# qiukunlong/seeksv

Measured on AMD Instinct MI355X. Metric: BAM records/sec through getclip+getsv, higher is better.
Workload: dtype i32/u8 (fp64 match-rate compare)

## Files before the change

### include/seeksv_hip.h

```cpp
#ifndef SEEKSV_HIP_H_
#define SEEKSV_HIP_H_

#include <stddef.h>
#include <stdint.h>

#ifdef __cplusplus
extern "C" {
#endif

#define SSV_ABI_VERSION 9

typedef enum {
	SSV_OK = 0,
	SSV_E_NODEVICE = -1,
	SSV_E_HIP = -2,
	SSV_E_ARG = -3,
	SSV_E_STATE = -4,
	SSV_E_NOMEM = -5,
	SSV_E_RANGE = -6
} ssv_status;

typedef enum {
	SSV_MEM_HOST = 0,
	SSV_MEM_DEVICE = 1,
	SSV_MEM_PERSISTENT = 2
} ssv_mem;

typedef struct {
	int32_t tid, pos;
	uint16_t flag;
	uint8_t mapq;
	uint8_t xc;
	uint16_t n_cigar;
	uint16_t pad;
	int32_t l_qseq, mtid, mpos, isize;
	uint32_t cigar_off;
	uint32_t cigar_head[5];
	uint64_t seq_off;
} ssv_record;

#define SSV_NO_SEQ UINT64_MAX
typedef struct {
	int64_t n;
	int32_t mem;
	int32_t max_ref_span;
	const int32_t *tid;
	const int32_t *pos;
	const uint16_t *flag;
	const uint8_t *mapq;
	const uint16_t *n_cigar;
	const int32_t *l_qseq;
	const int32_t *mtid;
	const int32_t *mpos;
	const int32_t *isize;
	const uint32_t *cigar_off;
	const uint32_t *cigar;
	const uint8_t *xc;
	const uint64_t *seq_off;
	const uint8_t *seqqual;
	int64_t n_cigar_total;
	int64_t seqqual_bytes;
	const ssv_record *rec;
	const uint8_t *cigar_ends;
	const struct ssv_tid_run *tid_runs;
	int64_t n_tid_runs;
} ssv_batch_t;

typedef struct ssv_tid_run { int64_t first; int32_t tid; int32_t pad; } ssv_tid_run;

typedef struct ssv_ctx ssv_ctx;


int ssv_ctx_create(int device, ssv_ctx **out);
void ssv_ctx_destroy(ssv_ctx *ctx);
int ssv_sync(ssv_ctx *ctx);
const char *ssv_last_error(const ssv_ctx *ctx);
int ssv_abi_version(void);
int ssv_device_count(void);
void *ssv_stream(ssv_ctx *ctx);

int ssv_host_alloc(size_t bytes, void **p);
int ssv_host_free(void *p);
int ssv_host_register(void *p, size_t bytes);
int ssv_host_unregister(void *p);
int ssv_host_bind_near(void *p, size_t bytes, int device);
int ssv_batch_prefetch(ssv_ctx *ctx, const ssv_batch_t *b);
int ssv_batch_prefetch_drop(ssv_ctx *ctx);

int ssv_batch_retain(ssv_ctx *ctx, const ssv_batch_t *device_batch, ssv_batch_t *out);
int ssv_batch_release(ssv_ctx *ctx, ssv_batch_t *retained);


typedef struct {
	double match_rate;
	int32_t min_mapq;
	int32_t save_low_quality;
	int32_t use_ownership;
	int32_t initial_last_tid;
	int32_t own_lo_tid, own_lo_pos;
	int32_t own_hi_tid, own_hi_pos;
} ssv_clip_params;

int ssv_clip_begin(ssv_ctx *ctx, const ssv_clip_params *p);
int ssv_clip_scan(ssv_ctx *ctx, const ssv_batch_t *b);
int ssv_clip_scan_range(ssv_ctx *ctx, const ssv_batch_t *b, int64_t rec_begin, int64_t rec_end);
int ssv_clip_event_count(ssv_ctx *ctx, int64_t *n_events);

typedef struct {
	int32_t tid;
	uint8_t side;
	uint8_t pad[3];
	int64_t first;
} ssv_table_run;

typedef struct {
	int64_t n_clusters;
	int64_t n_events;
	const int32_t *tid;
	const int32_t *pos;
	const uint8_t *side;
	const int32_t *support;
	const int32_t *left_len;
	const int32_t *right_len;
	const uint8_t *qual_missing;
	const uint64_t *str_off;
	const uint8_t *str;
	const uint64_t *cigar_off;
	const int32_t *n_cigar;
	const uint32_t *cigar;
	int32_t seq_packed;
	int32_t qual_bits;
	uint8_t qual_alphabet[64];
	int32_t format;
	int32_t base_bits;
	int32_t len_bytes, support_bytes, ncig_bytes;
	int32_t qual_group;
	const void *c_len;
	const void *c_support;
	const void *c_ncig;
	const uint8_t *c_flags;
	const ssv_table_run *runs;
	int64_t n_runs;
	const uint64_t *base_exc;
	int64_t n_base_exc;
	uint64_t str_bytes;
	uint64_t cigar_ops;
	int64_t support_sum;
	const void *c_cigar;
	int32_t cigar_bytes, pad4;
} ssv_cluster_table;

int ssv_clip_table_format(ssv_ctx *ctx, int format);
int ssv_clip_table_expand(ssv_ctx *ctx, ssv_cluster_table *t, int32_t n_threads);
uint64_t ssv_table_block_bytes3(int64_t n_bases, int32_t base_bits, int32_t qual_bits);
uint64_t ssv_table_block_bytes3g(int64_t n_bases, int32_t base_bits, int32_t qual_bits, int32_t qual_group);
uint64_t ssv_table_block_bytes(int32_t left_len, int32_t right_len);

int ssv_clip_cluster(ssv_ctx *ctx, ssv_cluster_table *out);
int ssv_clip_cluster_async(ssv_ctx *ctx, int64_t *n_clusters, int64_t *n_events);
int ssv_clip_table_wait(ssv_ctx *ctx, ssv_cluster_table *out);
int ssv_clip_table_wait_prev(ssv_ctx *ctx, ssv_cluster_table *out);


int ssv_isize_begin(ssv_ctx *ctx, int32_t min_mapq, int64_t max_pairs);
int ssv_isize_accumulate(ssv_ctx *ctx, const ssv_batch_t *b, int32_t *done);
int ssv_isize_finish(ssv_ctx *ctx, int64_t *n_pairs, int32_t *mean, int32_t *sd);


typedef struct {
	int32_t up_tid;
	int32_t down_tid;
	int32_t up_pos;
	int32_t down_pos;
	int32_t beg;
	int32_t end;
	uint8_t up_strand;
	uint8_t down_strand;
	uint8_t pad[2];
} ssv_junction;

typedef struct {
	int32_t tid;
	int32_t beg;
	int32_t end;
} ssv_interval;

typedef struct {
	const ssv_junction *junctions;
	int64_t n_junctions;
	int32_t mean, sd, times;
	int32_t disc_min_mapq;
	const ssv_interval *windows;
	int64_t n_windows;
	int32_t depth_min_mapq;
	int32_t n_targets;
	const int32_t *target_len;
} ssv_getsv_params;

int ssv_getsv_begin(ssv_ctx *ctx, const ssv_getsv_params *p);
int ssv_getsv_scan(ssv_ctx *ctx, const ssv_batch_t *b);
int ssv_getsv_prime(ssv_ctx *ctx, const ssv_batch_t *b, int32_t *sufficient);
int ssv_getsv_finish(ssv_ctx *ctx, int32_t *counts,
                     const ssv_interval *ranges, int64_t n_ranges, uint64_t *range_sum,
                     const ssv_interval *points, int64_t n_points, int32_t *point_depth,
                     int32_t *max_depth);

typedef struct ssv_group ssv_group;
int ssv_group_create(ssv_ctx **ctxs, int n, ssv_group **out);
void ssv_group_destroy(ssv_group *g);
int ssv_group_uses_rccl(const ssv_group *g);
int ssv_group_allgather(ssv_group *g, int rank, const void *send, size_t bytes, void *recv);


typedef struct {
	uint64_t c_off;
	uint32_t c_len;
	uint32_t u_len;
} ssv_bgzf_block;

typedef struct {
	int64_t n_records;
// ... 121 lines not shown
```

### seeksv_amd/_abi.py

```python
import ctypes as C
import os

import numpy as np

_HERE = os.path.dirname(os.path.abspath(__file__))
LIBDIR = os.environ.get("SSV_LIBDIR") or os.path.join(_HERE, "lib")

NO_SEQ = (1 << 64) - 1
MEM_HOST, MEM_DEVICE, MEM_PERSISTENT = 0, 1, 2
RECORD_DTYPE = np.dtype([("tid", np.int32), ("pos", np.int32), ("flag", np.uint16), ("mapq", np.uint8), ("xc", np.uint8), ("n_cigar", np.uint16), ("pad", np.uint16),
                         ("l_qseq", np.int32), ("mtid", np.int32), ("mpos", np.int32), ("isize", np.int32), ("cigar_off", np.uint32), ("cigar_head", np.uint32, (5,)),
                         ("seq_off", np.uint64)])
assert RECORD_DTYPE.itemsize == 64


class Batch(C.Structure):
    _fields_ = [
        ("n", C.c_int64), ("mem", C.c_int32), ("max_ref_span", C.c_int32),
        ("tid", C.c_void_p), ("pos", C.c_void_p), ("flag", C.c_void_p), ("mapq", C.c_void_p),
        ("n_cigar", C.c_void_p), ("l_qseq", C.c_void_p), ("mtid", C.c_void_p), ("mpos", C.c_void_p),
        ("isize", C.c_void_p), ("cigar_off", C.c_void_p), ("cigar", C.c_void_p), ("xc", C.c_void_p),
        ("seq_off", C.c_void_p), ("seqqual", C.c_void_p),
        ("n_cigar_total", C.c_int64), ("seqqual_bytes", C.c_int64),
        ("rec", C.c_void_p), ("cigar_ends", C.c_void_p),
        ("tid_runs", C.c_void_p), ("n_tid_runs", C.c_int64),
    ]

    def set_tid_runs(self, runs):
        if runs is None or len(runs) == 0:
            self.tid_runs, self.n_tid_runs, self._runs = None, 0, None
        else:
            self._runs = np.ascontiguousarray(runs, dtype=TID_RUN_DTYPE)
            self.tid_runs, self.n_tid_runs = self._runs.ctypes.data, len(self._runs)

    def get_tid_runs(self):
        if not self.tid_runs or self.n_tid_runs <= 0:
            return None
        return np.frombuffer((C.c_uint8 * (16 * self.n_tid_runs)).from_address(self.tid_runs), dtype=TID_RUN_DTYPE).copy()


TID_RUN_DTYPE = np.dtype([("first", np.int64), ("tid", np.int32), ("pad", np.int32)])


def runs_of_tid(tid):
    tid = np.asarray(tid)
    if tid.size == 0:
        return np.zeros(0, TID_RUN_DTYPE)
    starts = np.concatenate(([0], np.flatnonzero(tid[1:] != tid[:-1]) + 1))
    r = np.zeros(len(starts), TID_RUN_DTYPE)
    r["first"], r["tid"] = starts, tid[starts]
    return r


def rebase_runs(runs, first, n):
    if runs is None or len(runs) == 0 or n <= 0:
        return None
    k0 = int(np.searchsorted(runs["first"], first, side="right")) - 1
    k1 = int(np.searchsorted(runs["first"], first + n, side="left"))
    r = runs[k0:k1].copy()
    r["first"] = np.maximum(r["first"] - first, 0)
    return r


BATCH_FIELDS = [
    ("tid", np.int32), ("pos", np.int32), ("flag", np.uint16), ("mapq", np.uint8), ("n_cigar", np.uint16),
    ("l_qseq", np.int32), ("mtid", np.int32), ("mpos", np.int32), ("isize", np.int32),
    ("cigar_off", np.uint32), ("cigar", np.uint32), ("xc", np.uint8), ("seq_off", np.uint64), ("seqqual", np.uint8),
    ("cigar_ends", np.uint8),
]


class ClipParams(C.Structure):
    _fields_ = [("match_rate", C.c_double), ("min_mapq", C.c_int32), ("save_low_quality", C.c_int32),
                ("use_ownership", C.c_int32), ("initial_last_tid", C.c_int32), ("own_lo_tid", C.c_int32), ("own_lo_pos", C.c_int32),
                ("own_hi_tid", C.c_int32), ("own_hi_pos", C.c_int32)]

    @classmethod
    def make(cls, match_rate=0.9, min_mapq=1, save_low_quality=False, own=None, initial_last_tid=0):
        p = cls(match_rate, min_mapq, int(save_low_quality), 0, initial_last_tid, 0, 0, 0, 0)
        if own is not None:
            p.use_ownership = 1
            (p.own_lo_tid, p.own_lo_pos), (p.own_hi_tid, p.own_hi_pos) = own
        return p


class ClusterTable(C.Structure):
    _fields_ = [
        ("n_clusters", C.c_int64), ("n_events", C.c_int64),
        ("tid", C.POINTER(C.c_int32)), ("pos", C.POINTER(C.c_int32)), ("side", C.POINTER(C.c_uint8)),
        ("support", C.POINTER(C.c_int32)), ("left_len", C.POINTER(C.c_int32)), ("right_len", C.POINTER(C.c_int32)),
        ("qual_missing", C.POINTER(C.c_uint8)), ("str_off", C.POINTER(C.c_uint64)), ("str", C.POINTER(C.c_uint8)),
        ("cigar_off", C.POINTER(C.c_uint64)), ("n_cigar", C.POINTER(C.c_int32)), ("cigar", C.POINTER(C.c_uint32)),
    ]


class OrcClusterTable(C.Structure):
    _fields_ = ClusterTable._fields_ + [("str_bytes", C.c_int64), ("cigar_ops", C.c_int64)]


class HipClusterTable(C.Structure):
    _fields_ = ClusterTable._fields_ + [("seq_packed", C.c_int32), ("qual_bits", C.c_int32), ("qual_alphabet", C.c_uint8 * 64),
                                        ("format", C.c_int32), ("base_bits", C.c_int32), ("len_bytes", C.c_int32), ("support_bytes", C.c_int32), ("ncig_bytes", C.c_int32),
                                        ("qual_group", C.c_int32), ("c_len", C.c_void_p), ("c_support", C.c_void_p), ("c_ncig", C.c_void_p), ("c_flags", C.c_void_p),
                                        ("runs", C.c_void_p), ("n_runs", C.c_int64), ("base_exc", C.c_void_p), ("n_base_exc", C.c_int64), ("str_bytes", C.c_uint64),
                                        ("cigar_ops", C.c_uint64), ("support_sum", C.c_int64), ("c_cigar", C.c_void_p), ("cigar_bytes", C.c_int32), ("pad4", C.c_int32)]


TABLE_RUN_DTYPE = np.dtype([("tid", "<i4"), ("side", "u1"), ("pad", "u1", (3,)), ("first", "<i8")])


class Junction(C.Structure):
    _fields_ = [
        ("up_tid", C.c_int32), ("down_tid", C.c_int32), ("up_pos", C.c_int32), ("down_pos", C.c_int32),
        ("beg", C.c_int32), ("end", C.c_int32), ("up_strand", C.c_uint8), ("down_strand", C.c_uint8), ("pad", C.c_uint8 * 2),
    ]


JUNCTION_DTYPE = np.dtype([
    ("up_tid", np.int32), ("down_tid", np.int32), ("up_pos", np.int32), ("down_pos", np.int32),
    ("beg", np.int32), ("end", np.int32), ("up_strand", np.uint8), ("down_strand", np.uint8), ("pad", np.uint8, (2,)),
])
INTERVAL_DTYPE = np.dtype([("tid", np.int32), ("beg", np.int32), ("end", np.int32)])
assert JUNCTION_DTYPE.itemsize == C.sizeof(Junction) == 28
assert INTERVAL_DTYPE.itemsize == 12


class GetsvParams(C.Structure):
    _fields_ = [
        ("junctions", C.c_void_p), ("n_junctions", C.c_int64),
        ("mean", C.c_int32), ("sd", C.c_int32), ("times", C.c_int32), ("disc_min_mapq", C.c_int32),
        ("windows", C.c_void_p), ("n_windows", C.c_int64),
        ("depth_min_mapq", C.c_int32), ("n_targets", C.c_int32), ("target_len", C.c_void_p),
    ]


class JunctionIn(C.Structure):
    _fields_ = [("up_chr", C.c_char_p), ("down_chr", C.c_char_p), ("up_pos", C.c_int32), ("down_pos", C.c_int32),
                ("up_strand", C.c_char), ("down_strand", C.c_char)]


class Names(C.Structure):
    _fields_ = [("mem", C.c_int32), ("pad", C.c_int32), ("bias", C.c_int64), ("base", C.c_void_p), ("off", C.c_void_p), ("bytes", C.c_int64)]


class AlnCols(C.Structure):
    _fields_ = [("n", C.c_int64), ("n_cigar_total", C.c_int64), ("name_bytes", C.c_int64), ("tid", C.c_void_p), ("pos", C.c_void_p), ("flag", C.c_void_p),
                ("n_cigar", C.c_void_p), ("mapq", C.c_void_p), ("cigar_off", C.c_void_p), ("cigar", C.c_void_p), ("name_off", C.c_void_p), ("names", C.c_void_p),
                ("name_hash", C.c_void_p)]


class RtParams(C.Structure):
    _fields_ = [("min_mapq", C.c_int32), ("n_targets", C.c_int32), ("name_rank", C.POINTER(C.c_int32))]


class RtPair(C.Structure):
    _fields_ = [("up_tid", C.c_int32), ("up_pos", C.c_int32), ("down_tid", C.c_int32), ("down_pos", C.c_int32),
                ("up_strand", C.c_int8), ("down_strand", C.c_int8), ("kind", C.c_int16), ("microhomology", C.c_int32),
                ("up_left_clipped", C.c_int32), ("up_right_clipped", C.c_int32), ("down_left_clipped", C.c_int32), ("down_right_clipped", C.c_int32),
                ("up_len", C.c_int32), ("down_len", C.c_int32), ("up_cig_n", C.c_int32), ("down_cig_n", C.c_int32),
                ("up_cig_edit", C.c_int32), ("down_cig_edit", C.c_int32), ("seq_off", C.c_uint64), ("cig_off", C.c_uint64),
                ("first_record", C.c_int64), ("second_record", C.c_int64)]


class RtResult(C.Structure):
    _fields_ = [("n_pairs", C.c_int64), ("n_candidates", C.c_int64), ("pairs", C.POINTER(RtPair)), ("seqs", C.c_void_p), ("cigars", C.POINTER(C.c_uint32))]


def make_batch(arrays, mem=MEM_HOST, n=None):
    b = Batch()
    keep = []
    for name, dt in BATCH_FIELDS:
        a = arrays.get(name)
        if a is None:
            setattr(b, name, None)
            continue
        if isinstance(a, np.ndarray):
            a = np.ascontiguousarray(a, dtype=dt)
            keep.append(a)
            setattr(b, name, a.ctypes.data if a.size else None)
        else:
            setattr(b, name, int(a))
    rec = arrays.get("rec")
    if isinstance(rec, np.ndarray):
        rec = np.ascontiguousarray(rec)
        assert rec.nbytes == 64 * (len(arrays["tid"]) if n is None else n)
        keep.append(rec)
        b.rec = rec.ctypes.data if rec.size else None
    else:
        b.rec = int(rec) if rec else None
    b.mem = mem
    b.max_ref_span = int(arrays.get("max_ref_span", 0))
    if n is None:
        n = len(arrays["tid"])
    b.n = int(n)
# ... 175 lines not shown
```

### seeksv_amd/csrc/bamdec_api.inc

```

struct ssv_bamdec_state {
	int32_t n_targets = 0;
	uint64_t start = 0;
	int32_t prev_tid = 0;
	uint64_t carry = 0;
	std::vector<uint64_t> htokoff;
	uint64_t limit = UINT64_MAX;
	bool verify_crc = false;
	bool any_order = false;
	DBuf crc_tab;
	uint64_t expect_inflated = 0;
	DBuf inf_scratch, inf_dbg, tokens, tok_off, n_tok, carrybuf, comp, blocks, u_off, stream, status, chain, count, base, rec_off, stitch, tile_last, tile_prev, runs, small;
	DBuf raw_runs; HBuf h_raw_runs; std::vector<ssv_tid_run> tid_runs;
	DBuf tlen; bool have_tlen = false;
	DecodedColumns cols;
	DBuf rel, stash, seq_list, raw_bytes, raw_off, raw;
	HBuf h_stage[3], h_small, h_raw[2], h_runs, h_status;
	int raw_flip = 0;
	struct CompSlot {
		DBuf buf;
		const void *host = nullptr;
		size_t bytes = 0;
		hipEvent_t up = nullptr;
		hsa_signal_t up_sig{};
// ... 162 lines not shown
		CHECK(ensure_up(d.status, (size_t)n_blocks * 4));
		{
			ProfScope up(c, P_BAM_UPLOAD, (int64_t)comp_bytes);
			if (from) { if (from->via_link) { link_wait(c, from->up_sig); link_timed(c, from->up_sig, from->bytes, false); } else HIPCHECK(c, hipStreamWaitEvent(st, from->up, 0)); }
			else {
				bool done = false;
				if (c->link.ok && link_host_ok(comp) && (d.own_sig.handle || c->link.signal_create(0, 0, nullptr, &d.own_sig) == HSA_STATUS_SUCCESS)) {
					HIPCHECK(c, hipStreamSynchronize(st));
					c->link.signal_store(d.own_sig, 1);
					if (link_copy(c, d.comp.p, comp, comp_bytes, false, d.own_sig)) { link_wait(c, d.own_sig); link_timed(c, d.own_sig, comp_bytes, false); done = true; }
					else c->link.signal_store(d.own_sig, 0);
				}
				if (!done) HIPCHECK(c, hipMemcpyAsync(d.comp.p, comp, comp_bytes, hipMemcpyHostToDevice, st));
			}
			HIPCHECK(c, hipMemcpyAsync(d.blocks.p, d.hblocks.data(), (size_t)n_blocks * sizeof(ssv::BgzfBlock), hipMemcpyHostToDevice, st));
			HIPCHECK(c, hipMemcpyAsync(d.u_off.p, d.huoff.data(), ((size_t)n_blocks + 1) * 8, hipMemcpyHostToDevice, st));
		}
		ProfScope ps(c, P_BAM_INFLATE, (int64_t)(total - d.carry));
		const size_t n_waves = (size_t)((n_blocks + WAVE - 1) / WAVE);
		CHECK(ensure_up(d.inf_scratch, (n_waves + 8) * ssv::INFLATE_SCRATCH_BYTES));
		{
			d.htokoff.resize((size_t)n_blocks + 1);
			uint64_t words = 0;
			for (int64_t b = 0; b < n_blocks; ++b) { d.htokoff[(size_t)b] = words; words += ssv::token_capacity(blocks[b].u_len); }
			d.htokoff[(size_t)n_blocks] = words;
			CHECK(ensure_up(d.tokens, (size_t)words * 4 + 64)); CHECK(ensure_up(d.tok_off, ((size_t)n_blocks + 1) * 8)); CHECK(ensure_up(d.n_tok, (size_t)n_blocks * 4 + 16));
			HIPCHECK(c, hipMemcpyAsync(d.tok_off.p, d.htokoff.data(), ((size_t)n_blocks + 1) * 8, hipMemcpyHostToDevice, st));
			const size_t lds = ((size_t)ssv::INFLATE_LDS_BYTES / 64 + ssv::TOKENS_WINDOW + ssv::TOKENS_BASE_BYTES) * (size_t)WAVE;
			static const int tokens_mode = []() { const char *e = getenv("SSV_TOKENS"); return !e ? 0 : !strcmp(e, "wave") ? 1 : !strcmp(e, "lanes") ? 2 : 0; }();
			const bool tokens_wave = tokens_mode == 1 || (tokens_mode == 0 && n_blocks <= 65536);
			if (tokens_wave) {
				static const bool tw_phases = getenv("SSV_INFLATE_PHASES") != nullptr;
				unsigned long long *tw_dbg = nullptr;
				if (tw_phases) { CHECK(ensure_up(d.inf_dbg, 16 * 8)); HIPCHECK(c, hipMemsetAsync(d.inf_dbg.p, 0, 16 * 8, st)); tw_dbg = P<unsigned long long>(d.inf_dbg); }
				if (tw_phases)
					hipLaunchKernelGGL(ssv::k_bgzf_tokens_wave<true>, dim3((unsigned)n_blocks), dim3(WAVE), 0, st, comp_dev, P<ssv::BgzfBlock>(d.blocks), P<uint64_t>(d.u_off), P<uint64_t>(d.tok_off), n_blocks,
					                   P<uint8_t>(d.stream), P<uint32_t>(d.tokens), P<uint32_t>(d.n_tok), P<int>(d.status), tw_dbg);
				else
					hipLaunchKernelGGL(ssv::k_bgzf_tokens_wave<false>, dim3((unsigned)n_blocks), dim3(WAVE), 0, st, comp_dev, P<ssv::BgzfBlock>(d.blocks), P<uint64_t>(d.u_off), P<uint64_t>(d.tok_off), n_blocks,
					                   P<uint8_t>(d.stream), P<uint32_t>(d.tokens), P<uint32_t>(d.n_tok), P<int>(d.status), tw_dbg);
				if (tw_phases) {
					unsigned long long h[16];
					HIPCHECK(c, hipMemcpyAsync(h, tw_dbg, sizeof(h), hipMemcpyDeviceToHost, st));
					HIPCHECK(c, hipStreamSynchronize(st));
					const double nb = (double)n_blocks, win = (double)std::max<unsigned long long>(h[1], 1);
					fprintf(stderr, "[tokens wave] %lld BGZF blocks: %.2f deflate blocks and %.1f windows each; %.2f extra decode rounds per window, %.1f lanes decoding in rounds after the second per window; "
					        "most rounds in one window %llu; cycles per BGZF block: window loads %.0f, headers + tables %.0f, first round %.0f, later rounds %.0f, count + emit %.0f\n", (long long)n_blocks, h[0] / nb, h[1] / nb, h[2] / win, h[3] / win,
					        h[9], h[4] / nb, h[5] / nb, h[6] / nb, h[7] / nb, h[8] / nb);
					fprintf(stderr, "[tokens wave] symbols per lane in a window's first round: the busiest lane %.1f, the average lane %.1f\n", (double)h[10] / win, (double)h[11] / win / 64.0);
				}
			} else
				hipLaunchKernelGGL((ssv::k_bgzf_tokens<WAVE>), dim3((unsigned)n_waves), dim3(WAVE), lds, st, comp_dev, P<ssv::BgzfBlock>(d.blocks), P<uint64_t>(d.u_off), P<uint64_t>(d.tok_off), n_blocks,
				                   P<uint8_t>(d.stream), P<uint32_t>(d.tokens), P<uint32_t>(d.n_tok), P<int>(d.status), P<uint8_t>(d.inf_scratch));
			ProfScope pr(c, P_BAM_RESOLVE, (int64_t)(total - d.carry));
			static const bool resolve_win = []() { const char *e = getenv("SSV_RESOLVE"); return !e || strcmp(e, "wave") != 0; }();
			if (resolve_win) {
				static const bool rw_phases = getenv("SSV_INFLATE_PHASES") != nullptr;
				if (rw_phases) {
					CHECK(ensure_up(d.inf_dbg, 16 * 8)); HIPCHECK(c, hipMemsetAsync(d.inf_dbg.p, 0, 16 * 8, st));
					hipLaunchKernelGGL(ssv::k_bgzf_resolve_win<true>, dim3((unsigned)((n_blocks + WAVES_PER_BLOCK - 1) / WAVES_PER_BLOCK)), dim3(BLOCK), 0, st, P<uint32_t>(d.tokens), P<uint64_t>(d.tok_off), P<uint32_t>(d.n_tok),
					                   P<uint64_t>(d.u_off), P<ssv::BgzfBlock>(d.blocks), n_blocks, P<uint8_t>(d.stream), P<unsigned long long>(d.inf_dbg));
					unsigned long long h[16];
					HIPCHECK(c, hipMemcpyAsync(h, d.inf_dbg.p, sizeof(h), hipMemcpyDeviceToHost, st));
					HIPCHECK(c, hipStreamSynchronize(st));
					const double r = (double)std::max<unsigned long long>(h[0], 1);
					fprintf(stderr, "[resolve win] %lld BGZF blocks, %.1f rounds each; per round: %.1f tokens, %.2f phases, %.2f all-lanes matches, %.3f window moves; cycles per round: window %.0f, dependencies %.0f, "
					        "own-lane copies %.0f, all-lanes copies %.0f, store + rest %.0f\n", (long long)n_blocks, r / (double)n_blocks, h[3] / r, h[1] / r, h[2] / r, h[4] / r, h[5] / r, h[6] / r, h[7] / r, h[8] / r, h[9] / r);
				} else
					hipLaunchKernelGGL(ssv::k_bgzf_resolve_win<false>, dim3((unsigned)((n_blocks + WAVES_PER_BLOCK - 1) / WAVES_PER_BLOCK)), dim3(BLOCK), 0, st, P<uint32_t>(d.tokens), P<uint64_t>(d.tok_off), P<uint32_t>(d.n_tok),
					                   P<uint64_t>(d.u_off), P<ssv::BgzfBlock>(d.blocks), n_blocks, P<uint8_t>(d.stream), (unsigned long long *)nullptr);
			}
			else
				hipLaunchKernelGGL(ssv::k_bgzf_resolve_wave, dim3((unsigned)((n_blocks + WAVES_PER_BLOCK - 1) / WAVES_PER_BLOCK)), dim3(BLOCK), 0, st, P<uint32_t>(d.tokens), P<uint64_t>(d.tok_off), P<uint32_t>(d.n_tok),
				                   P<uint64_t>(d.u_off), n_blocks, P<uint8_t>(d.stream));
		}
		if (d.verify_crc) {
			if (!d.crc_tab.p) {
				std::unique_ptr<ssv::CrcTab> hp(new ssv::CrcTab);
				ssv::CrcTab &h = *hp;
				auto mult = [](uint32_t a, uint32_t b) { uint32_t m = 1u << 31, p = 0; for (;;) { if (a & m) { p ^= b; if ((a & (m - 1u)) == 0) break; } m >>= 1; b = (b & 1u) ? (b >> 1) ^ 0xedb88320u : b >> 1; } return p; };
				for (uint32_t i = 0; i < 256; ++i) { uint32_t v = i; for (int k = 0; k < 8; ++k) v = (v & 1u) ? (v >> 1) ^ 0xedb88320u : v >> 1; h.slice[0][i] = v; }
				for (int k = 1; k < 4; ++k) for (uint32_t i = 0; i < 256; ++i) h.slice[k][i] = (h.slice[k - 1][i] >> 8) ^ h.slice[0][h.slice[k - 1][i] & 0xffu];
				uint32_t p = 1u << 30;
				h.x2n[0] = p;
				for (int k = 1; k < 32; ++k) h.x2n[k] = p = mult(p, p);
				h.xr[0] = 1u << 31;
				for (int r = 1; r < 16; ++r) h.xr[r] = mult(h.xr[r - 1], h.x2n[3]);
				h.w16[0] = 1u << 31;
				for (int m = 1; m <= 128; ++m) h.w16[m] = mult(h.w16[m - 1], h.x2n[7]);
				const uint32_t x1k = h.w16[64];
				for (int k = 0; k < 4; ++k) for (uint32_t i = 0; i < 256; ++i) h.adv[k][i] = mult(x1k, i << (8 * k));
				CHECK(ensure(c, d.crc_tab, sizeof(h)));
				HIPCHECK(c, hipMemcpyAsync(d.crc_tab.p, &h, sizeof(h), hipMemcpyHostToDevice, st));
				HIPCHECK(c, hipStreamSynchronize(st));
			}
			hipLaunchKernelGGL(ssv::k_bgzf_crc, dim3((unsigned)n_blocks), dim3(WAVE), 0, st, comp_dev, P<ssv::BgzfBlock>(d.blocks), P<uint64_t>(d.u_off), n_blocks, P<uint8_t>(d.stream),
			                   P<ssv::CrcTab>(d.crc_tab), P<int>(d.status));
		}
		if (from) { HIPCHECK(c, hipEventRecord(from->done, st)); from->read = true; from->host = nullptr; }
	}
	d.info.n_records = 0; d.info.unmapped_raw = nullptr; d.info.unmapped_bytes = 0; d.info.n_tid_runs = 0; d.info.tid_run_index = nullptr; d.info.tid_run_tid = nullptr;
	d.info.inflated_bytes = total - d.carry;
	if (n_blocks == 0) {
		if (d.carry) { c->err = "truncated BAM record"; return SSV_E_ARG; }
		return SSV_OK;
	}
	const int64_t n_units = n_blocks * ssv::UNITS_PER_BLOCK;
	CHECK(ensure_up(d.chain, (size_t)n_units * sizeof(ssv::BlockChain)));
	CHECK(ensure_up(d.rel, (size_t)((n_units + 63) / 64) * ssv::REL_CAP * 64 * 2 + 64));
	CHECK(ensure_up(d.count, (size_t)n_units * 4 + 16)); CHECK(ensure_up(d.base, (size_t)n_units * 4 + 16));
	CHECK(ensure_up(d.stitch, sizeof(ssv::StitchOut))); CHECK(ensure_up(d.small, 256));
	CHECK(ensure_host(c, d.h_small, 256)); CHECK(ensure_host(c, d.h_status, (size_t)n_blocks * 4));
	CHECK(ensure_up(c->scan_scratch, (size_t)scan_scratch_elems(std::max<int64_t>(n_units, (int64_t)(total / 36 + 1))) * 8 + 64));
	CHECK(ensure_up(c->scan_scratch64, (size_t)scan_scratch_elems((int64_t)(total / 36 + 1)) * 8 + 64));
	{
		ProfScope ps(c, P_BAM_RECORDS, n_blocks);
		hipLaunchKernelGGL(ssv::k_find_records, dim3((unsigned)((n_units + BLOCK - 1) / BLOCK)), dim3(BLOCK), 0, st, P<uint8_t>(d.stream), P<ssv::BgzfBlock>(d.blocks), P<uint64_t>(d.u_off), n_units,
		                   d.start, stream_end, d.n_targets, d.have_tlen ? P<int32_t>(d.tlen) : (const int32_t *)nullptr, P<ssv::BlockChain>(d.chain), P<uint16_t>(d.rel));
		HIPCHECK(c, hipMemsetAsync(d.stitch.p, 0, sizeof(ssv::StitchOut), st));
		hipLaunchKernelGGL(ssv::k_stitch_check, dim3((unsigned)((n_units + BLOCK - 1) / BLOCK)), dim3(BLOCK), 0, st, P<ssv::BgzfBlock>(d.blocks), P<uint64_t>(d.u_off), n_units, d.start, stream_end, P<ssv::BlockChain>(d.chain),
		                   P<uint32_t>(d.count), P<ssv::StitchOut>(d.stitch));
		hipLaunchKernelGGL(ssv::k_stitch_blocks, dim3(1), dim3(WAVE), 0, st, P<uint8_t>(d.stream), P<ssv::BgzfBlock>(d.blocks), P<uint64_t>(d.u_off), n_units, d.start, stream_end,
		                   P<ssv::BlockChain>(d.chain), P<uint32_t>(d.count), P<ssv::StitchOut>(d.stitch));
		exclusive_scan<uint32_t, uint32_t>(st, P<uint32_t>(d.count), P<uint32_t>(d.base), n_units, 0u, P<uint32_t>(c->scan_scratch), (uint32_t *)nullptr);
	}
	HIPCHECK(c, hipMemcpyAsync(d.h_small.p, d.stitch.p, sizeof(ssv::StitchOut), hipMemcpyDeviceToHost, st));
	HIPCHECK(c, hipMemcpyAsync(d.h_status.p, d.status.p, (size_t)n_blocks * 4, hipMemcpyDeviceToHost, st));
	HIPCHECK(c, hipStreamSynchronize(st));
	for (int64_t b = 0; b < n_blocks; ++b)
		if (P<int>(d.h_status)[b] != 0) {
			c->err = P<int>(d.h_status)[b] == ssv::INF_E_CRC ? "BGZF block " + std::to_string(b) + " of the chunk: CRC32 mismatch (its bytes are not what was written)"
			                                                 : "BGZF inflate failed (block " + std::to_string(b) + " of the chunk, code " + std::to_string(P<int>(d.h_status)[b]) + ")";
			return SSV_E_ARG;
		}
	const ssv::StitchOut so = *P<ssv::StitchOut>(d.h_small);
	if (so.corrupt) { c->err = "corrupt BAM record"; return SSV_E_ARG; }
	const int64_t n = so.n_records;
	d.info.n_records = n; d.info.repaired_blocks = so.n_repaired; d.info.tail_offset = so.tail;
	d.carry = stream_end - so.tail; d.start = 0;
	if (d.carry) {
		CHECK(ensure_up(d.carrybuf, (size_t)d.carry + 64));
		HIPCHECK(c, hipMemcpyAsync(d.carrybuf.p, P<uint8_t>(d.stream) + so.tail, d.carry, hipMemcpyDeviceToDevice, st));
	}
	if (n == 0) return SSV_OK;
	const size_t N = (size_t)n;
	CHECK(ensure_up(d.rec_off, N * 8 + 16));
	CHECK(d.cols.reserve(c, N, up));
	CHECK(ensure_up(d.stash, N * 8 + 16)); CHECK(ensure_up(d.seq_list, N * 4 + 16)); CHECK(ensure_up(d.raw_bytes, N * 4 + 16)); CHECK(ensure_up(d.raw_off, N * 8 + 16));
	const int64_t n_tiles = (n + BLOCK - 1) / BLOCK;
	CHECK(ensure_up(d.tile_last, (size_t)n_tiles * 4)); CHECK(ensure_up(d.tile_prev, (size_t)n_tiles * 4));
	const uint32_t run_cap = 1u << 16;
	CHECK(ensure_up(d.runs, (size_t)run_cap * sizeof(ssv::TidRun)));
	constexpr uint32_t RAW_RUN_CAP = 64;
	CHECK(ensure_up(d.raw_runs, (size_t)RAW_RUN_CAP * sizeof(ssv::TidRun))); CHECK(ensure_host(c, d.h_raw_runs, (size_t)RAW_RUN_CAP * sizeof(ssv::TidRun)));
	HIPCHECK(c, hipMemsetAsync(d.small.p, 0, 256, st));
	uint32_t *sm = P<uint32_t>(d.small);
	{
		ProfScope ps(c, P_BAM_DECODE, n);
		hipLaunchKernelGGL(ssv::k_list_records, dim3((unsigned)((n_units + BLOCK - 1) / BLOCK)), dim3(BLOCK), 0, st, P<uint8_t>(d.stream), P<ssv::BlockChain>(d.chain), P<uint32_t>(d.count),
		                   P<uint32_t>(d.base), n_units, P<uint16_t>(d.rel), P<uint64_t>(d.rec_off));
		const ssv::RecColumns rc{P<uint32_t>(d.raw_bytes), P<uint2>(d.stash), reinterpret_cast<int32_t *>(sm), sm + 1};
		hipLaunchKernelGGL(ssv::k_record_fields, dim3((unsigned)((n + BLOCK - 1) / BLOCK)), dim3(BLOCK), 0, st, P<uint8_t>(d.stream), P<uint64_t>(d.rec_off), n, keep_all_seq, d.cols.view(), rc);
		d.cols.layout(st, n, P<uint32_t>(c->scan_scratch), P<uint64_t>(c->scan_scratch64), sm + 4, reinterpret_cast<uint64_t *>(sm + 6));
		exclusive_scan<uint32_t, uint64_t>(st, P<uint32_t>(d.raw_bytes), P<uint64_t>(d.raw_off), n, 0ull, P<uint64_t>(c->scan_scratch64), reinterpret_cast<uint64_t *>(sm + 8));
	}
	HIPCHECK(c, hipMemcpyAsync(d.h_small.p, d.small.p, 64, hipMemcpyDeviceToHost, st));
	HIPCHECK(c, hipStreamSynchronize(st));
	uint64_t seq_total, raw_total;
	const uint32_t cigar_total = P<uint32_t>(d.h_small)[4];
	memcpy(&seq_total, P<uint32_t>(d.h_small) + 6, 8); memcpy(&raw_total, P<uint32_t>(d.h_small) + 8, 8);
	if (P<uint32_t>(d.h_small)[1]) { c->err = "corrupt BAM record"; return SSV_E_ARG; }
	CHECK(d.cols.reserve_variable(c, cigar_total, (size_t)seq_total, up)); CHECK(ensure_up(d.raw, (size_t)raw_total + 64));
	const ssv::DecodedCols col = d.cols.view();
	{
		ProfScope ps(c, P_BAM_DECODE, n);
		hipLaunchKernelGGL(ssv::k_record_cigars, dim3((unsigned)((n + BLOCK * ssv::CIGARS_PER_THREAD - 1) / (BLOCK * ssv::CIGARS_PER_THREAD))), dim3(BLOCK), 0, st, P<uint8_t>(d.stream), P<uint64_t>(d.rec_off), n, col.n_cigar,
		                   col.cigar_off, P<uint2>(d.stash), col.seq_bytes, col.xc, col.seq_off, col.cigar, P<uint32_t>(d.seq_list), sm + 10);
		hipLaunchKernelGGL(ssv::k_record_seqs, dim3((unsigned)std::min<int64_t>((n * 16 + BLOCK - 1) / BLOCK, 2048)), dim3(BLOCK), 0, st, P<uint8_t>(d.stream), P<uint64_t>(d.rec_off),
		                   col.n_cigar, col.seq_bytes, col.seq_off, P<uint32_t>(d.seq_list), sm + 10, col.seqqual, col.xc);
		hipLaunchKernelGGL(ssv::k_raw_copy, dim3((unsigned)((n + BLOCK - 1) / BLOCK)), dim3(BLOCK), 0, st, P<uint8_t>(d.stream), P<uint64_t>(d.rec_off), n, P<uint32_t>(d.raw_bytes), P<uint64_t>(d.raw_off), P<uint8_t>(d.raw));
		hipLaunchKernelGGL(ssv::k_tid_tile_last, dim3((unsigned)n_tiles), dim3(BLOCK), 0, st, col.tid, col.flag, n, P<int32_t>(d.tile_last));
		hipLaunchKernelGGL(ssv::k_tid_tile_carry, dim3(1), dim3(WAVE), 0, st, P<int32_t>(d.tile_last), n_tiles, d.prev_tid, P<int32_t>(d.tile_prev), reinterpret_cast<int32_t *>(sm + 3));
		hipLaunchKernelGGL(ssv::k_tid_runs, dim3((unsigned)n_tiles), dim3(BLOCK), 0, st, col.tid, col.flag, n, P<int32_t>(d.tile_prev), P<ssv::TidRun>(d.runs), run_cap, sm + 2);
		hipLaunchKernelGGL(ssv::k_tid_raw_runs, dim3((unsigned)n_tiles), dim3(BLOCK), 0, st, col.tid, n, P<ssv::TidRun>(d.raw_runs), RAW_RUN_CAP, sm + 11);
		HIPCHECK(c, hipMemcpyAsync(d.h_raw_runs.p, d.raw_runs.p, (size_t)RAW_RUN_CAP * sizeof(ssv::TidRun), hipMemcpyDeviceToHost, st));
	}
	HIPCHECK(c, hipMemcpyAsync(d.h_small.p, d.small.p, 64, hipMemcpyDeviceToHost, st));
	HIPCHECK(c, hipStreamSynchronize(st));
	const uint32_t *hs = P<uint32_t>(d.h_small);
	uint32_t n_runs = hs[2];
	if (n_runs > run_cap) {
		if (!d.any_order) { c->err = "more than 65536 contig changes in one chunk: the BAM is not coordinate sorted"; return SSV_E_ARG; }
		n_runs = 0;
	}
	d.prev_tid = (int32_t)hs[3];
	CHECK(ensure_host(c, d.h_runs, (size_t)n_runs * sizeof(ssv::TidRun) + 64 + (size_t)n_runs * 8));
	HBuf &h_raw = d.h_raw[d.raw_flip ^= 1];
	CHECK(ensure_host(c, h_raw, (size_t)raw_total + 64));
	if (n_runs) HIPCHECK(c, hipMemcpyAsync(d.h_runs.p, d.runs.p, (size_t)n_runs * sizeof(ssv::TidRun), hipMemcpyDeviceToHost, st));
	if (raw_total) HIPCHECK(c, hipMemcpyAsync(h_raw.p, d.raw.p, (size_t)raw_total, hipMemcpyDeviceToHost, st));
	if (n_runs || raw_total) HIPCHECK(c, hipStreamSynchronize(st));
	{
		ssv::TidRun *r = P<ssv::TidRun>(d.h_runs);
		std::sort(r, r + n_runs, [](const ssv::TidRun &a, const ssv::TidRun &b) { return a.index < b.index; });
		uint32_t *idx = reinterpret_cast<uint32_t *>(P<uint8_t>(d.h_runs) + (((size_t)n_runs * sizeof(ssv::TidRun) + 63) & ~(size_t)63));
		int32_t *tv = reinterpret_cast<int32_t *>(idx + n_runs);
		for (uint32_t k = 0; k < n_runs; ++k) { idx[k] = r[k].index; tv[k] = r[k].tid; }
		d.info.n_tid_runs = n_runs; d.info.tid_run_index = idx; d.info.tid_run_tid = tv;
	}
	d.info.unmapped_raw = P<uint8_t>(h_raw); d.info.unmapped_bytes = raw_total; d.info.last_tid = d.prev_tid;
	d.cols.fill(out, n, (int64_t)cigar_total, (int64_t)seq_total);
	out->max_ref_span = (int32_t)hs[0] > 0 ? (int32_t)hs[0] : 1;
	{
		const uint32_t nr = hs[11];
		d.tid_runs.clear();
		if (nr >= 1 && nr <= RAW_RUN_CAP) {
			const ssv::TidRun *r = P<ssv::TidRun>(d.h_raw_runs);
			for (uint32_t k = 0; k < nr; ++k) d.tid_runs.push_back(ssv_tid_run{(int64_t)r[k].index, r[k].tid, 0});
			std::sort(d.tid_runs.begin(), d.tid_runs.end(), [](const ssv_tid_run &a, const ssv_tid_run &b) { return a.first < b.first; });
			out->tid_runs = d.tid_runs.data(); out->n_tid_runs = (int64_t)nr;
		}
	}
	return SSV_OK;
}

int ssv_bamdec_names(ssv_ctx *c, ssv_names_t *out)
{
	if (!c || !out) return SSV_E_ARG;
	if (!c->bd) { c->err = "ssv_bamdec_names before ssv_bamdec_begin"; return SSV_E_STATE; }
	memset(out, 0, sizeof(*out));
	out->mem = SSV_MEM_DEVICE; out->bias = 36;
	out->base = P<char>(c->bd->stream); out->off = P<uint64_t>(c->bd->rec_off);
	return SSV_OK;
}

int ssv_bamdec_last(ssv_ctx *c, ssv_bamdec_info *info)
{
	if (!c || !c->bd || !info) return SSV_E_ARG;
	*info = c->bd->info;
	return SSV_OK;
}
```

### seeksv_amd/csrc/bamdec_kernels.h

```cpp
#pragma once

#include "batch_columns.h"
#include "common.h"
#include "inflate_core.h"
#include "resolve_wave.h"
#include "inflate_wave.h"

namespace ssv {

constexpr uint32_t BD_NONE = 0xffffffffu;

template <int STRIDE> struct LdsTabT {
	uint8_t *lit8; uint32_t *hi; uint8_t *dst8;
	uint8_t *len8; uint16_t *off16;
	int lane;
	static constexpr int stride = STRIDE;
	__device__ __forceinline__ uint16_t lit_get(int i) const { return (uint16_t)(lit8[i * stride + lane] | (((hi[(i >> 5) * stride + lane] >> (i & 31)) & 1u) << 8)); }
	__device__ __forceinline__ void lit_set(int i, uint16_t v)
	{
		lit8[i * stride + lane] = (uint8_t)v;
		uint32_t &w = hi[(i >> 5) * stride + lane];
		w = (w & ~(1u << (i & 31))) | ((uint32_t)(v >> 8) << (i & 31));
	}
	__device__ __forceinline__ uint16_t dst_get(int i) const { return dst8[i * stride + lane]; }
// ... 416 lines not shown
	else {
		int s = 0;
		for (uint32_t k = 0; k < ncig; ++k) {
			const uint32_t op = ld_u32(r + o_cig + 4ull * k);
			const uint32_t t = op & 15u;
			if (k == 0) first2.x = op;
			if (k == 1) first2.y = op;
			if (t == 0 || t == 2 || t == 3 || t == 7 || t == 8) s += (int)(op >> 4);
			if ((k == 0 || k == ncig - 1) && t == 4) soft = true;
			if (k == 0) ends = t | (t << 4);
			if (k == ncig - 1) ends = (ends & 15u) | (t << 4);
		}
		if (s > span) span = s;
		c.seq_bytes[i] = (soft || keep_all_seq) ? (uint32_t)(((uint64_t)l_seq + 1) / 2 + (uint64_t)l_seq) : 0u;
		x.raw_bytes[i] = (flag & (F_UNMAP | F_MUNMAP)) ? 4u + bs : 0u;
	}
	c.cigar_ends[i] = (uint8_t)ends;
	x.stash[i] = first2;
	c.xc[i] = soft ? 2 : 0;
	return span;
}

__global__ __launch_bounds__(BLOCK) void k_record_fields(const uint8_t *__restrict__ u, const uint64_t *__restrict__ rec_off, int64_t n, int keep_all_seq, DecodedCols c, RecColumns x)
{
	const int64_t i = (int64_t)blockIdx.x * BLOCK + threadIdx.x;
	int span = 1;
	if (i < n) span = record_fields_of(u + rec_off[i], i, keep_all_seq, c, x);
	span = wave_max(span);
	if (lane_id() == 0 && span > 1 && span > __hip_atomic_load(x.max_span, __ATOMIC_RELAXED, __HIP_MEMORY_SCOPE_AGENT)) atomicMax(x.max_span, span);
}

__device__ __forceinline__ int aux_xc_flag(const uint8_t *p, const uint8_t *end)
{
	while (p + 3 <= end) {
		const uint8_t t0 = p[0], t1 = p[1], ty = p[2];
		p += 3;
		const bool hit = t0 == 'X' && t1 == 'C';
		int64_t v = 0;
		uint32_t sz;
		switch (ty) {
		case 'A': case 'c': sz = 1; if (hit && ty == 'c') v = (int8_t)p[0]; break;
		case 'C': sz = 1; if (hit) v = p[0]; break;
		case 's': sz = 2; if (hit) v = (int16_t)ld_u16(p); break;
		case 'S': sz = 2; if (hit) v = ld_u16(p); break;
		case 'i': sz = 4; if (hit) v = ld_i32(p); break;
		case 'I': sz = 4; if (hit) v = ld_u32(p); break;
		case 'f': sz = 4; break;
		case 'd': sz = 8; break;
		case 'Z': case 'H': { const uint8_t *q = p; while (q < end && *q) ++q; sz = (uint32_t)(q - p) + 1; break; }
		case 'B': {
			if (p + 5 > end) return 0;
			const uint8_t st = p[0];
			const uint32_t cnt = ld_u32(p + 1);
			const uint32_t es = (st == 'c' || st == 'C') ? 1 : (st == 's' || st == 'S') ? 2 : 4;
			sz = 5 + cnt * es;
			break;
		}
		default: return 0;
		}
		if (p + sz > end) return 0;
		if (hit) return v != 0;
		p += sz;
	}
	return 0;
}

constexpr int CIGARS_PER_THREAD = 16;
__global__ __launch_bounds__(BLOCK) void k_record_cigars(const uint8_t *__restrict__ u, const uint64_t *__restrict__ rec_off, int64_t n, const uint16_t *__restrict__ n_cigar,
                                                        const uint32_t *__restrict__ cigar_off, const uint2 *__restrict__ stash, const uint32_t *__restrict__ seq_bytes,
                                                        const uint8_t *__restrict__ xc, uint64_t *__restrict__ seq_off, uint32_t *__restrict__ cigar, uint32_t *__restrict__ list,
                                                        uint32_t *__restrict__ n_list)
{
	__shared__ uint32_t mine[BLOCK * CIGARS_PER_THREAD];
	__shared__ uint32_t n_mine, base;
	if (threadIdx.x == 0) n_mine = 0;
	__syncthreads();
	const int64_t i0 = (int64_t)blockIdx.x * (BLOCK * CIGARS_PER_THREAD);
	for (int t = 0; t < CIGARS_PER_THREAD; ++t) {
		const int64_t i = i0 + (int64_t)t * BLOCK + threadIdx.x;
		bool has = false;
		if (i < n) {
			const uint32_t ncig = n_cigar[i], co = cigar_off[i];
			if (ncig <= 2u) {
				const uint2 f = stash[i];
				if (ncig > 0u) cigar[co] = f.x;
				if (ncig > 1u) cigar[co + 1] = f.y;
			} else {
				const uint8_t *r = u + rec_off[i] + 4;
				const uint64_t o_cig = 32ull + r[8];
				for (uint32_t k = 0; k < ncig; ++k) cigar[co + k] = ld_u32(r + o_cig + 4ull * k);
			}
			const bool ships = seq_bytes[i] != 0u;
			if (!ships) seq_off[i] = ~0ull;
			has = ships || xc[i] == 2;
		}
		const uint64_t m = __ballot(has);
		if (m) {
			const int leader = __ffsll((long long)m) - 1;
			uint32_t at = 0;
			if (lane_id() == leader) at = atomicAdd(&n_mine, (uint32_t)__popcll(m));
			at = (uint32_t)__shfl((int)at, leader);
			if (has) mine[at + (uint32_t)__popcll(m & ((1ull << lane_id()) - 1ull))] = (uint32_t)i;
		}
	}
	__syncthreads();
	if (threadIdx.x == 0 && n_mine) base = atomicAdd(n_list, n_mine);
	__syncthreads();
	for (uint32_t k = threadIdx.x; k < n_mine; k += BLOCK) list[base + k] = mine[k];
}

__global__ __launch_bounds__(BLOCK) void k_record_seqs(const uint8_t *__restrict__ u, const uint64_t *__restrict__ rec_off, const uint16_t *__restrict__ n_cigar,
                                                      const uint32_t *__restrict__ seq_bytes, const uint64_t *__restrict__ seq_off, const uint32_t *__restrict__ list,
                                                      const uint32_t *__restrict__ n_list, uint8_t *__restrict__ seqqual, uint8_t *__restrict__ xc)
{
	const uint32_t total = *n_list;
	const int sub = (int)(threadIdx.x & 15);
	for (uint32_t e = (blockIdx.x * BLOCK + threadIdx.x) >> 4; e < total; e += gridDim.x * (BLOCK / 16)) {
		const uint32_t i = list[e];
		const uint8_t *r = u + rec_off[i] + 4;
		const uint32_t bs = ld_u32(r - 4), l_name = r[8], ncig = n_cigar[i];
		const uint64_t o_seq = 32ull + l_name + 4ull * ncig;
		const uint32_t sb = seq_bytes[i];
		if (sb) {
			const uint64_t so = seq_off[i];
			for (uint32_t k = (uint32_t)sub; k < sb; k += 16) seqqual[so + k] = r[o_seq + k];
		}
		if (sub == 0 && xc[i] == 2) {
			const int32_t l_seq = ld_i32(r + 16);
			xc[i] = (uint8_t)aux_xc_flag(r + o_seq + ((uint64_t)l_seq + 1) / 2 + (uint64_t)l_seq, r + bs);
		}
	}
}

__global__ __launch_bounds__(BLOCK) void k_raw_copy(const uint8_t *__restrict__ u, const uint64_t *__restrict__ rec_off, int64_t n, const uint32_t *__restrict__ raw_bytes,
                                                   const uint64_t *__restrict__ raw_off, uint8_t *__restrict__ raw)
{
	const int64_t i = (int64_t)blockIdx.x * BLOCK + threadIdx.x;
	const uint32_t nb = i < n ? raw_bytes[i] : 0u;
	uint64_t m = __ballot(nb != 0u);
	while (m) {
		const int l = __ffsll((long long)m) - 1;
		m &= m - 1;
		const uint32_t knb = (uint32_t)__shfl((int)nb, l);
		const int64_t ki = i - lane_id() + l;
		const uint8_t *r = u + rec_off[ki];
		const uint64_t o = raw_off[ki];
		for (uint32_t k = (uint32_t)lane_id(); k < knb; k += WAVE) raw[o + k] = r[k];
	}
}

struct TidRun { uint32_t index; int32_t tid; };
constexpr int32_t TID_NONE = INT32_MIN;

__global__ __launch_bounds__(BLOCK) void k_tid_raw_runs(const int32_t *__restrict__ tid, int64_t n, TidRun *__restrict__ runs, uint32_t cap, uint32_t *__restrict__ count)
{
	const int64_t i = (int64_t)blockIdx.x * BLOCK + threadIdx.x;
	if (i >= n) return;
	const int32_t t = tid[i];
	if (i == 0 || tid[i - 1] != t) {
		const uint32_t k = atomicAdd(count, 1u);
		if (k < cap) { runs[k].index = (uint32_t)i; runs[k].tid = t; }
	}
}


__global__ __launch_bounds__(BLOCK) void k_tid_tile_last(const int32_t *__restrict__ tid, const uint16_t *__restrict__ flag, int64_t n, int32_t *__restrict__ tile_last)
{
	__shared__ int lds[WAVES_PER_BLOCK];
	const int64_t i = (int64_t)blockIdx.x * BLOCK + threadIdx.x;
	const bool q = i < n && !(flag[i] & (F_UNMAP | F_MUNMAP));
	int idx = wave_max(q ? (int)threadIdx.x : -1);
	if (lane_id() == 0) lds[wave_id()] = idx;
	__syncthreads();
	if (threadIdx.x == 0) {
		int m = -1;
		for (int w = 0; w < WAVES_PER_BLOCK; ++w) m = lds[w] > m ? lds[w] : m;
		tile_last[blockIdx.x] = m >= 0 ? tid[(int64_t)blockIdx.x * BLOCK + m] : TID_NONE;
	}
}

__global__ __launch_bounds__(WAVE) void k_tid_tile_carry(const int32_t *__restrict__ tile_last, int64_t n_tiles, int32_t prev_tid, int32_t *__restrict__ tile_prev, int32_t *__restrict__ last_tid)
{
	int32_t cur = prev_tid;
	constexpr int AHEAD = 16;
	for (int64_t base0 = 0; base0 < n_tiles; base0 += WAVE * AHEAD) {
	int32_t vals[AHEAD];
#pragma unroll
	for (int j = 0; j < AHEAD; ++j) { const int64_t t = base0 + (int64_t)j * WAVE + lane_id(); vals[j] = t < n_tiles ? tile_last[t] : TID_NONE; }
#pragma unroll
	for (int j = 0; j < AHEAD; ++j) {
		const int64_t t = base0 + (int64_t)j * WAVE + lane_id();
		const int32_t mine = vals[j];
		const uint64_t have = __ballot(mine != TID_NONE);
		const uint64_t below = have & lanemask_lt();
		const int src = below ? 63 - __clzll((long long)below) : 0;
		const int32_t got = __shfl(mine, src, 64);
		if (t < n_tiles) tile_prev[t] = below ? got : cur;
		if (have) cur = __shfl(mine, 63 - __clzll((long long)have), 64);
	}
	}
	if (lane_id() == 0) *last_tid = cur;
}

__global__ __launch_bounds__(BLOCK) void k_tid_runs(const int32_t *__restrict__ tid, const uint16_t *__restrict__ flag, int64_t n, const int32_t *__restrict__ tile_prev,
                                                   TidRun *__restrict__ runs, uint32_t cap, uint32_t *__restrict__ n_runs)
{
	__shared__ int32_t wave_last[WAVES_PER_BLOCK];
	const int64_t i = (int64_t)blockIdx.x * BLOCK + threadIdx.x;
	const bool q = i < n && !(flag[i] & (F_UNMAP | F_MUNMAP));
	const int32_t mine = q ? tid[i] : TID_NONE;
	const uint64_t have = __ballot(q);
	const int32_t top = __shfl(mine, have ? 63 - __clzll((long long)have) : 0, 64);
	if (lane_id() == 0) wave_last[wave_id()] = have ? top : TID_NONE;
	const uint64_t below = have & lanemask_lt();
	int32_t before = __shfl(mine, below ? 63 - __clzll((long long)below) : 0, 64);
	__syncthreads();
	if (!below) {
		before = tile_prev[blockIdx.x];
		for (int w = 0; w < wave_id(); ++w) if (wave_last[w] != TID_NONE) before = wave_last[w];
	}
	if (q && mine != before) {
		const uint32_t k = atomicAdd(n_runs, 1u);
		if (k < cap) { runs[k].index = (uint32_t)i; runs[k].tid = mine; }
	}
}

}
```

### seeksv_amd/csrc/getsv_api.inc

```

struct ssv_getsv_state {
	bool active = false;
	ssv_getsv_params p{};
	std::vector<DevJunction> junc;
	std::vector<ssv_interval> win;
	std::vector<int32_t> tlen;
	std::vector<int64_t> ctg_tile_off;
	int32_t map_span = -1;
	int32_t wmax = 0;
	int64_t diff_len = 0;
	DBuf djunc, counts, wtid, wbeg, wend, woff, diff, tilemap, tile_win, tile_junc, ctgoff, maxdepth, span;
	DBuf q_tid, q_out64;
	DBuf dense_list, cap_flags, cap_deep, cap_carry, cap_ring, cap_ring_tmp, cap_tail[2][4];
	int32_t cap_tail_n = 0, cap_tail_cur = 0, cap_ring_mask = 0;
	HBuf h_q;
};

static int fill_runs(ssv_ctx *c, const ssv_batch_t *b, RunTab &R)
{
	memset(&R, 0, sizeof(R));
	if (!b->tid_runs || b->n_tid_runs <= 0 || b->n_tid_runs > RUN_MAX || getenv("SSV_NO_TID_RUNS")) return SSV_OK;
	const int64_t k = b->n_tid_runs;
	if (b->tid_runs[0].first != 0) { c->err = "tid_runs must start at record 0"; return SSV_E_ARG; }
	for (int64_t i = 0; i < k; ++i) {
		if (i && b->tid_runs[i].first <= b->tid_runs[i - 1].first) { c->err = "tid_runs must be strictly increasing"; return SSV_E_ARG; }
		if (b->tid_runs[i].first >= b->n) { c->err = "tid_runs reach past the batch"; return SSV_E_ARG; }
		R.first[i] = b->tid_runs[i].first; R.tid[i] = b->tid_runs[i].tid;
	}
	R.first[k] = b->n; R.n = (int32_t)k;
	return SSV_OK;
}

static int gs_build_tilemap(ssv_ctx *c, int32_t span)
{
	ssv_getsv_state &G = *c->getsv;
	const size_t ntile = (size_t)G.ctg_tile_off.back();
	CHECK(ensure(c, G.tilemap, ntile + 16)); CHECK(ensure(c, G.tile_win, ntile * 4 + 16)); CHECK(ensure(c, G.tile_junc, ntile * 4 + 16));
	HIPCHECK(c, hipMemsetAsync(G.tilemap.p, 0, ntile + 16, c->st));
	const int64_t nw = (int64_t)G.win.size(), nj = (int64_t)G.junc.size();
	if (nw) k_tile_mark_windows<<<grid_for(nw, BLOCK), BLOCK, 0, c->st>>>(P<int32_t>(G.wtid), P<int32_t>(G.wbeg), P<int32_t>(G.wend), nw, span, P<int64_t>(G.ctgoff),
	                                                                        G.p.n_targets, P<uint32_t>(G.tilemap), P<uint32_t>(G.tile_win));
	if (nj) k_tile_mark_junctions<<<grid_for(nj, BLOCK), BLOCK, 0, c->st>>>(P<DevJunction>(G.djunc), nj, span, G.wmax, P<int64_t>(G.ctgoff), G.p.n_targets,
	                                                                          P<uint32_t>(G.tilemap), P<uint32_t>(G.tile_junc));
	HIPCHECK(c, hipGetLastError());
	G.map_span = span;
	return SSV_OK;
}

int ssv_getsv_begin(ssv_ctx *c, const ssv_getsv_params *p)
{
	if (!c || !p || p->n_targets < 0 || p->n_junctions < 0 || p->n_windows < 0) return SSV_E_ARG;
	ssv_getsv_state &G = *c->getsv;
	if ((p->n_targets && !p->target_len) || (p->n_junctions && !p->junctions) || (p->n_windows && !p->windows)) return SSV_E_ARG;
	c->pf.clear();
	HIPCHECK(c, hipSetDevice(c->device));
	G.p = *p;
	G.tlen.assign(p->target_len, p->target_len + p->n_targets);
	G.ctg_tile_off.assign((size_t)p->n_targets + 1, 0);
	for (int t = 0; t < p->n_targets; ++t) G.ctg_tile_off[(size_t)t + 1] = G.ctg_tile_off[(size_t)t] + ((int64_t)std::max(0, G.tlen[(size_t)t]) >> TILE_SHIFT) + 1;
	G.map_span = -1;
	G.junc.clear();
	G.wmax = 0;
	for (int64_t k = 0; k < p->n_junctions; ++k) {
		const ssv_junction &s = p->junctions[k];
		DevJunction j;
		j.up_tid = s.up_tid; j.down_tid = s.down_tid; j.up_pos = s.up_pos; j.down_pos = s.down_pos; j.beg = s.beg; j.end = s.end;
		j.up_strand = s.up_strand; j.down_strand = s.down_strand; j.pad = 0; j.orig = (int32_t)k;
		G.junc.push_back(j);
		if ((int64_t)s.end - s.beg > G.wmax) G.wmax = (int32_t)std::min<int64_t>((int64_t)s.end - s.beg, 0x7fffffff);
	}
	std::stable_sort(G.junc.begin(), G.junc.end(), [](const DevJunction &a, const DevJunction &b) { return a.up_tid != b.up_tid ? a.up_tid < b.up_tid : a.beg < b.beg; });
	G.win.assign(p->windows, p->windows + p->n_windows);
	for (size_t k = 0; k < G.win.size(); ++k) {
		const ssv_interval &w = G.win[k];
		if (w.end < w.beg || (k && (G.win[k - 1].tid > w.tid || (G.win[k - 1].tid == w.tid && G.win[k - 1].end >= w.beg)))) {
			c->err = "depth windows must be sorted, disjoint and non-empty"; return SSV_E_ARG;
		}
	}
	const size_t nj = G.junc.size(), nw = G.win.size();
	std::vector<int32_t> wt(nw), wb(nw), we(nw);
	std::vector<int64_t> wo(nw + 1, 0);
	for (size_t k = 0; k < nw; ++k) { wt[k] = G.win[k].tid; wb[k] = G.win[k].beg; we[k] = G.win[k].end; wo[k + 1] = wo[k] + ((int64_t)we[k] - wb[k] + 1) + 1; }
	G.diff_len = wo[nw];
	CHECK(ensure(c, G.djunc, nj * sizeof(DevJunction) + 16)); CHECK(ensure(c, G.counts, nj * 4 + 16));
	CHECK(ensure(c, G.wtid, nw * 4 + 16)); CHECK(ensure(c, G.wbeg, nw * 4 + 16)); CHECK(ensure(c, G.wend, nw * 4 + 16)); CHECK(ensure(c, G.woff, (nw + 1) * 8));
	CHECK(ensure(c, G.diff, (size_t)G.diff_len * 4 + 16)); CHECK(ensure(c, G.ctgoff, G.ctg_tile_off.size() * 8)); CHECK(ensure(c, G.maxdepth, 16));
	CHECK(ensure(c, G.span, 16));
	if (nj) HIPCHECK(c, hipMemcpyAsync(G.djunc.p, G.junc.data(), nj * sizeof(DevJunction), hipMemcpyHostToDevice, c->st));
	if (nw) {
		HIPCHECK(c, hipMemcpyAsync(G.wtid.p, wt.data(), nw * 4, hipMemcpyHostToDevice, c->st));
		HIPCHECK(c, hipMemcpyAsync(G.wbeg.p, wb.data(), nw * 4, hipMemcpyHostToDevice, c->st));
		HIPCHECK(c, hipMemcpyAsync(G.wend.p, we.data(), nw * 4, hipMemcpyHostToDevice, c->st));
	}
	HIPCHECK(c, hipMemcpyAsync(G.woff.p, wo.data(), (nw + 1) * 8, hipMemcpyHostToDevice, c->st));
	HIPCHECK(c, hipMemcpyAsync(G.ctgoff.p, G.ctg_tile_off.data(), G.ctg_tile_off.size() * 8, hipMemcpyHostToDevice, c->st));
	HIPCHECK(c, hipMemsetAsync(G.counts.p, 0, nj * 4 + 16, c->st));
	HIPCHECK(c, hipMemsetAsync(G.diff.p, 0, (size_t)G.diff_len * 4 + 16, c->st));
	HIPCHECK(c, hipMemsetAsync(G.maxdepth.p, 0, 16, c->st));
	CHECK(ensure(c, G.cap_carry, sizeof(CapCarry))); CHECK(ensure(c, G.cap_flags, 16));
	HIPCHECK(c, hipMemsetAsync(G.cap_carry.p, 0, sizeof(CapCarry), c->st));
	G.cap_tail_n = 0; G.cap_tail_cur = 0; G.cap_ring_mask = 0;
	HIPCHECK(c, hipStreamSynchronize(c->st));
	G.active = true;
	return SSV_OK;
}

static int cap_launches(ssv_ctx *c, const GetsvArgs &a, const DevBatch &d, int64_t ntiles, int prime)
{
	ssv_getsv_state &G = *c->getsv;
	ProfScope ps(c, P_GETSV_CAND, 0);
	if (G.cap_ring_mask == 0 || (int64_t)G.map_span + 2 > (int64_t)G.cap_ring_mask + 1) {
		int64_t e = CAP_LDS_RING;
		while (e < (int64_t)G.map_span + 2) e <<= 1;
		if (e > (1ll << 30)) { c->err = "reference span of a read beyond 2^30"; return SSV_E_RANGE; }
		if (G.cap_ring_mask == 0) CHECK(ensure(c, G.cap_ring, (size_t)e * 4));
		else {
			CHECK(ensure(c, G.cap_ring_tmp, (size_t)e * 4));
			HIPCHECK(c, hipMemsetAsync(G.cap_ring_tmp.p, 0, (size_t)e * 4, c->st));
			k_cap_regrow<<<64, BLOCK, 0, c->st>>>(P<CapCarry>(G.cap_carry), P<int32_t>(G.cap_ring), G.cap_ring_mask, P<int32_t>(G.cap_ring_tmp), (int32_t)(e - 1));
			HIPCHECK(c, hipGetLastError());
			std::swap(G.cap_ring, G.cap_ring_tmp);
		}
		G.cap_ring_mask = (int32_t)(e - 1);
	}
	CHECK(ensure(c, G.cap_deep, (size_t)ntiles + 16));
	for (int s_ = 0; s_ < 2; ++s_) { CHECK(ensure(c, G.cap_tail[s_][0], CAP_TAIL * 4)); CHECK(ensure(c, G.cap_tail[s_][1], CAP_TAIL * 4)); CHECK(ensure(c, G.cap_tail[s_][2], CAP_TAIL * 4)); CHECK(ensure(c, G.cap_tail[s_][3], CAP_TAIL)); }
	CapArgs ca;
	ca.g = a; ca.span = G.map_span; ca.prime = prime;
	DBuf *ot = G.cap_tail[G.cap_tail_cur], *nt = G.cap_tail[G.cap_tail_cur ^ 1];
	ca.tail_tid = P<int32_t>(ot[0]); ca.tail_pos = P<int32_t>(ot[1]); ca.tail_end = P<int32_t>(ot[2]); ca.tail_pass = P<uint8_t>(ot[3]); ca.tail_n = G.cap_tail_n;
	ca.deep = P<uint8_t>(G.cap_deep); ca.ntiles = ntiles; ca.flags = P<int>(G.cap_flags); ca.carry = P<CapCarry>(G.cap_carry);
	ca.ring = P<int32_t>(G.cap_ring); ca.ring_mask = G.cap_ring_mask;
	ca.ntail_tid = P<int32_t>(nt[0]); ca.ntail_pos = P<int32_t>(nt[1]); ca.ntail_end = P<int32_t>(nt[2]); ca.ntail_pass = P<uint8_t>(nt[3]);
	ca.ntail_n = (int32_t)std::min<int64_t>(CAP_TAIL, (int64_t)G.cap_tail_n + d.n);
	k_cap_mark<<<(unsigned)std::min<int64_t>(ntiles, 1024), BLOCK, 0, c->st>>>(ca);
	k_cap_sweep<<<1, WAVE, 0, c->st>>>(ca);
	k_cap_tail<<<grid_for(ca.ntail_n, BLOCK), BLOCK, 0, c->st>>>(ca);
	HIPCHECK(c, hipGetLastError());
	G.cap_tail_n = ca.ntail_n; G.cap_tail_cur ^= 1;
	return SSV_OK;
}

int ssv_getsv_scan(ssv_ctx *c, const ssv_batch_t *b)
{
	if (!c || !b) return SSV_E_ARG;
	ssv_getsv_state &G = *c->getsv;
	if (!G.active) { c->err = "ssv_getsv_scan before ssv_getsv_begin"; return SSV_E_STATE; }
	HIPCHECK(c, hipSetDevice(c->device));
	if (b->n == 0) return SSV_OK;
	DevBatch d;
	CHECK(stage_batch(c, b, d));
	if (!d.cigar) { c->err = "batch without cigar"; return SSV_E_ARG; }
	int32_t span = d.max_ref_span;
	if (span <= 0) {
		HIPCHECK(c, hipMemsetAsync(G.span.p, 0, 16, c->st));
		k_max_span<<<grid_for(d.n, BLOCK), BLOCK, 0, c->st>>>(d, P<int>(G.span));
		CHECK(ensure_host(c, c->h_totals, 64));
		HIPCHECK(c, hipMemcpyAsync(c->h_totals.p, G.span.p, 4, hipMemcpyDeviceToHost, c->st));
		HIPCHECK(c, hipStreamSynchronize(c->st));
		span = std::max(1, *P<int>(c->h_totals));
	}
	if (span > G.map_span) CHECK(gs_build_tilemap(c, span));
	GetsvArgs a;
	CHECK(fill_runs(c, b, a.runs));
	static const bool verify_runs = getenv("SSV_VERIFY_RUNS") && atoi(getenv("SSV_VERIFY_RUNS")) != 0;
	if (verify_runs && a.runs.n > 0) {
		CHECK(ensure(c, c->counters, sizeof(ClipCounters)));
		CHECK(ensure_host(c, c->h_counters, sizeof(ClipCounters)));
		HIPCHECK(c, hipMemsetAsync(c->counters.p, 0, sizeof(ClipCounters), c->st));
		k_verify_runs<<<(unsigned)std::min<int64_t>(256 * 8, (d.n + BLOCK * 4 - 1) / (BLOCK * 4)), BLOCK, 0, c->st>>>(d.tid, d.n, a.runs, &P<ClipCounters>(c->counters)->n_cand);
		HIPCHECK(c, hipGetLastError());
		HIPCHECK(c, hipMemcpyAsync(c->h_counters.p, c->counters.p, sizeof(ClipCounters), hipMemcpyDeviceToHost, c->st));
		HIPCHECK(c, hipStreamSynchronize(c->st));
		const unsigned long long badrec = P<ClipCounters>(c->h_counters)->n_cand;
		if (badrec) { c->err = "tid_runs disagree with the tid column at record " + std::to_string(badrec - 1) + " (SSV_VERIFY_RUNS)"; return SSV_E_ARG; }
	}
	a.b = d; a.tilemap = P<uint8_t>(G.tilemap); a.tile_win = P<uint32_t>(G.tile_win); a.tile_junc = P<uint32_t>(G.tile_junc); a.ctg_tile_off = P<int64_t>(G.ctgoff); a.n_targets = G.p.n_targets;
	a.junc = P<DevJunction>(G.djunc); a.n_junc = (int64_t)G.junc.size(); a.junc_wmax = G.wmax;
	a.mean = G.p.mean; a.sd = G.p.sd; a.times = G.p.times; a.disc_min_mapq = G.p.disc_min_mapq;
	a.min_ins = std::max(0, a.mean - a.sd * a.times); a.max_ins = a.mean + a.sd * a.times;
	a.counts = P<int32_t>(G.counts);
	a.win_tid = P<int32_t>(G.wtid); a.win_beg = P<int32_t>(G.wbeg); a.win_end = P<int32_t>(G.wend); a.win_off = P<int64_t>(G.woff);
	a.n_win = (int64_t)G.win.size(); a.depth_min_mapq = G.p.depth_min_mapq; a.diff = P<int32_t>(G.diff);
	a.cap_flag = nullptr; a.cap_span = G.map_span;
	HIPCHECK(c, hipMemsetAsync(G.cap_flags.p, 0, 16, c->st));
	if (a.n_win > 0) a.cap_flag = P<int>(G.cap_flags);
	const int64_t ntiles = (d.n + CS_TILE - 1) / CS_TILE;
	const unsigned grid = scan_blocks(ntiles, "SSV_GETSV_SCAN_BLOCKS", 256 * 4);
	CHECK(ensure(c, c->tile_cnt, ntiles * 4));
	CHECK(ensure(c, c->tile_off, ntiles * 4));
	CHECK(ensure(c, c->counters, sizeof(ClipCounters)));
	CHECK(ensure_host(c, c->h_counters, sizeof(ClipCounters)));
	if (c->stage_cap == 0) c->stage_cap = std::max<int64_t>(1 << 16, d.n / 8);
	ClipCounters *hc = P<ClipCounters>(c->h_counters);
	ClipCounters *dc = P<ClipCounters>(c->counters);
	GetsvStage g;
	for (int attempt = 0;; ++attempt) {
		const int64_t block_cap = (c->stage_cap + grid - 1) / grid;
		CHECK(ensure(c, c->stage, (size_t)block_cap * grid * 4));
		HIPCHECK(c, hipMemsetAsync(c->counters.p, 0, sizeof(ClipCounters), c->st));
		g.tile_cnt = P<uint32_t>(c->tile_cnt); g.tile_off = P<uint32_t>(c->tile_off); g.stage = P<uint32_t>(c->stage); g.block_cap = block_cap;
		g.overflow = &dc->overflow; g.ntiles = ntiles;
		g.dense_list = nullptr; g.dense_n = nullptr; g.n_cand = &dc->n_cand;
		{
			ProfScope ps(c, P_GETSV_SCAN, d.n);
			if (a.runs.n > 0 && d.n >= CS_TILE) k_getsv_scan_runs<<<grid, BLOCK, 0, c->st>>>(a, g);
			else k_getsv_scan<<<grid, BLOCK, 0, c->st>>>(a, g);
		}
		HIPCHECK(c, hipGetLastError());
		HIPCHECK(c, hipMemcpyAsync(hc, c->counters.p, sizeof(ClipCounters), hipMemcpyDeviceToHost, c->st));
		HIPCHECK(c, hipStreamSynchronize(c->st));
		if (!hc->overflow) break;
		if (attempt > 6) { c->err = "getsv staging overflow"; return SSV_E_HIP; }
		c->stage_cap *= 4;
	}
	{
		ProfScope ps(c, P_GETSV_CAND, d.n);
		const int64_t dense_max = std::min<int64_t>(ntiles, (int64_t)(hc->n_cand / GC_DENSE_MIN));
		if (dense_max > 0) {
			CHECK(ensure(c, G.dense_list, (size_t)dense_max * sizeof(DenseTile)));
			g.dense_list = P<DenseTile>(G.dense_list); g.dense_n = P<int>(G.cap_flags) + 2;
			k_dense_tiles<<<grid_for(ntiles, BLOCK), BLOCK, 0, c->st>>>(a, g);
		}
		k_getsv_cand<<<grid_for(ntiles, WAVES_PER_BLOCK), BLOCK, 0, c->st>>>(a, g);
		if (g.dense_list) k_getsv_cand_dense<<<(unsigned)dense_max, BLOCK, 0, c->st>>>(a, g);
	}
	HIPCHECK(c, hipGetLastError());
	if (a.n_win > 0) CHECK(cap_launches(c, a, d, ntiles, 0));
	return SSV_OK;
}

int ssv_getsv_prime(ssv_ctx *c, const ssv_batch_t *b, int32_t *sufficient)
{
	if (!c || !b || !sufficient) return SSV_E_ARG;
	ssv_getsv_state &G = *c->getsv;
	if (!G.active) { c->err = "ssv_getsv_prime before ssv_getsv_begin"; return SSV_E_STATE; }
	if (G.cap_tail_n != 0) { c->err = "ssv_getsv_prime after records were scanned"; return SSV_E_STATE; }
	HIPCHECK(c, hipSetDevice(c->device));
	*sufficient = 1;
	if (b->n == 0 || G.win.empty()) return SSV_OK;
	DevBatch d;
	CHECK(stage_batch(c, b, d));
	int32_t span = d.max_ref_span;
	if (span <= 0) {
		HIPCHECK(c, hipMemsetAsync(G.span.p, 0, 16, c->st));
		k_max_span<<<grid_for(d.n, BLOCK), BLOCK, 0, c->st>>>(d, P<int>(G.span));
		CHECK(ensure_host(c, c->h_totals, 128));
		HIPCHECK(c, hipMemcpyAsync(c->h_totals.p, G.span.p, 4, hipMemcpyDeviceToHost, c->st));
		HIPCHECK(c, hipStreamSynchronize(c->st));
		span = std::max(1, *P<int>(c->h_totals));
	}
	if (span > G.map_span) CHECK(gs_build_tilemap(c, span));
	GetsvArgs a;
	memset(&a, 0, sizeof(a));
	a.b = d; a.depth_min_mapq = G.p.depth_min_mapq; a.n_targets = G.p.n_targets; a.cap_span = G.map_span;
	a.tilemap = P<uint8_t>(G.tilemap); a.tile_win = P<uint32_t>(G.tile_win); a.ctg_tile_off = P<int64_t>(G.ctgoff);
	a.win_tid = P<int32_t>(G.wtid); a.win_beg = P<int32_t>(G.wbeg); a.win_end = P<int32_t>(G.wend); a.win_off = P<int64_t>(G.woff);
	a.n_win = (int64_t)G.win.size(); a.diff = P<int32_t>(G.diff);
	int one[4] = {1, 0, 0, 0};
	HIPCHECK(c, hipMemcpyAsync(G.cap_flags.p, one, 16, hipMemcpyHostToDevice, c->st));
	HIPCHECK(c, hipStreamSynchronize(c->st));
	const int64_t ntiles = (d.n + CS_TILE - 1) / CS_TILE;
	CHECK(cap_launches(c, a, d, ntiles, 1));
	CHECK(ensure_host(c, c->h_totals, 128));
	const int64_t nt = std::min<int64_t>(ntiles, 4);
	HIPCHECK(c, hipMemcpyAsync(c->h_totals.p, G.cap_deep.p, (size_t)nt, hipMemcpyDeviceToHost, c->st));
	HIPCHECK(c, hipStreamSynchronize(c->st));
	for (int64_t t = 1; t < nt; ++t) if (P<uint8_t>(c->h_totals)[t]) *sufficient = 0;
	if (ntiles < 4) *sufficient = 0;
	return SSV_OK;
}

int ssv_getsv_finish(ssv_ctx *c, int32_t *counts, const ssv_interval *ranges, int64_t n_ranges, uint64_t *range_sum,
                     const ssv_interval *points, int64_t n_points, int32_t *point_depth, int32_t *max_depth)
{
	if (!c || n_ranges < 0 || n_points < 0 || (n_ranges && (!ranges || !range_sum)) || (n_points && (!points || !point_depth))) return SSV_E_ARG;
	ssv_getsv_state &G = *c->getsv;
	if (!G.active) { c->err = "ssv_getsv_finish before ssv_getsv_begin"; return SSV_E_STATE; }
	HIPCHECK(c, hipSetDevice(c->device));
	G.active = false;
	const int64_t nw = (int64_t)G.win.size(), nj = (int64_t)G.junc.size();
	ProfScope ps(c, P_DEPTH_FINISH, nw);
	if (nw) k_depth_prefix<<<grid_for(nw, WAVES_PER_BLOCK), BLOCK, 0, c->st>>>(P<int64_t>(G.woff), nw, P<int32_t>(G.diff), P<int32_t>(G.maxdepth));
	const size_t up_bytes = ((size_t)n_ranges * 3 + (size_t)n_points * 2) * 4;
	const size_t o_pd = (size_t)n_ranges * 8, o_cnt = o_pd + (size_t)n_points * 4, o_max = o_cnt + (size_t)nj * 4, down_bytes = o_max + 4;
	CHECK(ensure_host(c, G.h_q, up_bytes + down_bytes + 64));
	CHECK(ensure(c, G.q_tid, up_bytes + 16)); CHECK(ensure(c, G.q_out64, down_bytes + 16));
	int32_t *up = P<int32_t>(G.h_q);
	uint8_t *down = P<uint8_t>(G.h_q) + ((up_bytes + 15) & ~(size_t)15);
	int32_t *rt = up, *rb = rt + n_ranges, *re = rb + n_ranges, *pt = re + n_ranges, *pb = pt + n_points;
	for (int64_t k = 0; k < n_ranges; ++k) { rt[k] = ranges[k].tid; rb[k] = ranges[k].beg; re[k] = ranges[k].end; }
	for (int64_t k = 0; k < n_points; ++k) { pt[k] = points[k].tid; pb[k] = points[k].beg; }
	int32_t *d_up = P<int32_t>(G.q_tid);
	uint8_t *d_down = P<uint8_t>(G.q_out64);
	if (up_bytes) HIPCHECK(c, hipMemcpyAsync(d_up, up, up_bytes, hipMemcpyHostToDevice, c->st));
	if (n_ranges) k_range_sum<<<grid_for(n_ranges, WAVES_PER_BLOCK), BLOCK, 0, c->st>>>(P<int32_t>(G.wtid), P<int32_t>(G.wbeg), P<int32_t>(G.wend), P<int64_t>(G.woff), nw,
	                                                                                  P<int32_t>(G.diff), d_up, d_up + n_ranges, d_up + 2 * n_ranges, n_ranges,
	                                                                                  reinterpret_cast<unsigned long long *>(d_down));
	if (n_points) k_point_depth<<<grid_for(n_points, BLOCK), BLOCK, 0, c->st>>>(P<int32_t>(G.wtid), P<int32_t>(G.wbeg), P<int32_t>(G.wend), P<int64_t>(G.woff), nw,
	                                                                          P<int32_t>(G.diff), d_up + 3 * n_ranges, d_up + 3 * n_ranges + n_points, n_points,
	                                                                          reinterpret_cast<int32_t *>(d_down + o_pd));
	if (nj) HIPCHECK(c, hipMemcpyAsync(d_down + o_cnt, G.counts.p, (size_t)nj * 4, hipMemcpyDeviceToDevice, c->st));
	HIPCHECK(c, hipMemcpyAsync(d_down + o_max, G.maxdepth.p, 4, hipMemcpyDeviceToDevice, c->st));
	HIPCHECK(c, hipGetLastError());
	HIPCHECK(c, hipMemcpyAsync(down, d_down, down_bytes, hipMemcpyDeviceToHost, c->st));
	HIPCHECK(c, hipStreamSynchronize(c->st));
	if (n_ranges) memcpy(range_sum, down, (size_t)n_ranges * 8);
	if (n_points) memcpy(point_depth, down + o_pd, (size_t)n_points * 4);
	if (counts && nj) memcpy(counts, down + o_cnt, (size_t)nj * 4);
	if (max_depth) memcpy(max_depth, down + o_max, 4);
	return SSV_OK;
}
```

### seeksv_amd/csrc/getsv_kernels.h

```cpp
#pragma once

#include "clip_kernels.h"
#include "common.h"

namespace ssv {

__device__ __forceinline__ bool is_hard_clip(const DevBatch &b, const RecLine &r)
{
	const int n = r.n_cigar();
	if (n == 0) return false;
	return (r.head(0) & 15u) == C_H || (r.op(b.cigar, n - 1) & 15u) == C_H;
}


constexpr int ISZ_TILE = BLOCK;

__device__ __forceinline__ bool isize_qualifies(const DevBatch &b, const RecLine &r, int min_mapq)
{
	if (r.mapq() < min_mapq) return false;
	const int f = r.flag();
	if (!((f & F_PAIRED) && (f & F_PROPER) && !(f & F_DUP))) return false;
	if (r.isize() <= 0) return false;
	return !is_hard_clip(b, r);
}

__global__ __launch_bounds__(BLOCK) void k_isize_count(DevBatch b, int min_mapq, int32_t *__restrict__ val, uint32_t *__restrict__ tile_cnt)
{
	__shared__ uint32_t lds[WAVES_PER_BLOCK];
	const int q = (int)(threadIdx.x & 3);
	uint32_t c = 0;
#pragma unroll
	for (int k = 0; k < 4; ++k) {
		const int64_t i = (int64_t)blockIdx.x * ISZ_TILE + k * (BLOCK / 4) + (threadIdx.x >> 2);
		if (i < b.n) {
			const RecLine r = rec_load_quad(b.rec, i, q);
			const bool ok = isize_qualifies(b, r, min_mapq);
			if (q == 0) { val[i] = ok ? r.isize() : 0; c += ok ? 1u : 0u; }
		}
	}
	c = wave_sum(c);
	if (lane_id() == 0) lds[wave_id()] = c;
	__syncthreads();
	if (threadIdx.x == 0) tile_cnt[blockIdx.x] = lds[0] + lds[1] + lds[2] + lds[3];
}

__global__ __launch_bounds__(BLOCK) void k_isize_collect(const int32_t *__restrict__ val, int64_t n, const uint32_t *__restrict__ tile_base, int64_t count_before, int64_t max_pairs,
                                                         int32_t *__restrict__ vals)
{
	__shared__ uint32_t lds[WAVES_PER_BLOCK + 1];
	const int64_t i = (int64_t)blockIdx.x * ISZ_TILE + threadIdx.x;
	const int v = i < n ? val[i] : 0;
	uint32_t tot;
	const uint32_t ex = block_exclusive_sum(v > 0 ? 1u : 0u, lds, &tot);
	const int64_t o = count_before + tile_base[blockIdx.x] + ex;
	if (v > 0 && o < max_pairs) vals[o] = v;
}

__global__ __launch_bounds__(BLOCK) void k_isize_reduce(const int32_t *__restrict__ vals, int64_t n, int mode, const long long *__restrict__ mean_from, long long *__restrict__ acc)
{
	__shared__ long long lds[WAVES_PER_BLOCK];
	const int mean = mode ? (int)((unsigned long)*mean_from / (unsigned long)n) : 0;
	long long s = 0;
	for (int64_t i = (int64_t)blockIdx.x * blockDim.x + threadIdx.x; i < n; i += (int64_t)gridDim.x * blockDim.x) {
		int x = vals[i];
		if (mode == 0) s += x;
		else {
			int d = (int)((unsigned)x - (unsigned)mean);
			s += (int)((unsigned)d * (unsigned)d);
		}
	}
	s = wave_sum(s);
	if (lane_id() == 0) lds[wave_id()] = s;
	__syncthreads();
	if (threadIdx.x == 0) atomicAdd((unsigned long long *)acc, (unsigned long long)(lds[0] + lds[1] + lds[2] + lds[3]));
}


constexpr int TILE_SHIFT = 9;
constexpr uint8_t TM_DEPTH = 1, TM_JUNC = 2;

struct DevJunction {
	int32_t up_tid, down_tid, up_pos, down_pos, beg, end;
	uint8_t up_strand, down_strand;
	uint16_t pad;
	int32_t orig;
};

constexpr int RUN_MAX = 48;
struct RunTab {
	int32_t n;
	int32_t tid[RUN_MAX];
	int64_t first[RUN_MAX + 1];
};

struct GetsvArgs {
	DevBatch b;
	RunTab runs;
	const uint8_t *tilemap;
	const uint32_t *tile_win;
	const uint32_t *tile_junc;
	const int64_t *ctg_tile_off;
	int32_t n_targets;
	const DevJunction *junc;
	int64_t n_junc;
	int32_t junc_wmax;
	int32_t mean, sd, times, min_ins, max_ins, disc_min_mapq;
	int32_t *counts;
	const int32_t *win_tid, *win_beg, *win_end;
	const int64_t *win_off;
	int64_t n_win;
	int32_t depth_min_mapq;
	int32_t *diff;
	int *cap_flag;
	int32_t cap_span;
};

__device__ __forceinline__ bool is_concordant(int flag, int isize, int mean, int sd, int times)
{
	int lo = mean - sd * times, hi = mean + sd * times;
	if (!(flag & F_REV) && (flag & F_MREV) && lo <= isize && isize <= hi) return true;
	if ((flag & F_REV) && !(flag & F_MREV) && isize < 0) {
		int a = isize < 0 ? -isize : isize;
		return lo <= a && a <= hi;
	}
	return false;
}

__device__ __forceinline__ bool discordant_geometry(const DevJunction &j, int flag, int pos, int mpos, int lq, int mtid, int min_ins, int max_ins)
{
	if (!(j.down_tid != -1 && j.down_tid == mtid)) return false;
	const int K = 5;
	const int up = j.up_pos, down = j.down_pos;
	if (j.up_strand == '+' && j.down_strand == '+' && pos + lq <= up + K && mpos + 1 >= down - K) {
		if (!(flag & F_REV) && (flag & F_MREV)) {
			int ins = up - pos + mpos + lq - down + 1;
			if (j.up_tid == j.down_tid && up > down && up - down + 1 + 2 * lq <= max_ins) {
				while (ins <= max_ins) {
					if (ins >= min_ins) return true;
					ins += up - down + 1;
				}
				return false;
			}
			return min_ins <= ins && ins <= max_ins;
		}
		return false;
	} else if (j.up_strand == '-' && j.down_strand == '+' && (flag & F_REV) && (flag & F_MREV) && mpos + 1 >= down - K) {
		int ins = pos + 1 - up + 1 + mpos + lq - down + 1;
		return min_ins <= ins && ins <= max_ins;
	} else if (j.up_strand == '+' && j.down_strand == '-' && !(flag & F_REV) && !(flag & F_MREV) && pos + lq <= up + K && mpos + lq <= down + K) {
		int ins = up - pos + down - (mpos + lq) + 1;
		return min_ins <= ins && ins <= max_ins;
	}
	return false;
}

struct CandRec {
	int mapq, flag, isize, nc, mtid, mpos, lq;
	const uint32_t *cig;
	RecLine line;
};

__device__ __forceinline__ CandRec cand_load(const DevBatch &b, int64_t i)
{
	CandRec r;
	r.line = rec_load(b.rec, i);
	r.mapq = r.line.mapq(); r.flag = r.line.flag(); r.isize = r.line.isize(); r.nc = r.line.n_cigar(); r.mtid = r.line.mtid(); r.mpos = r.line.mpos(); r.lq = r.line.l_qseq();
	r.cig = b.cigar + r.line.cigar_off();
	return r;
}

__device__ __forceinline__ uint32_t cand_op(const CandRec &r, int k) { return k < 5 ? r.line.head(k) : r.cig[k]; }

__device__ __forceinline__ bool discordant_read(const GetsvArgs &a, const CandRec &r)
{
	if (r.mapq < a.disc_min_mapq) return false;
	const int flag = r.flag;
	if (flag & (F_DUP | F_UNMAP | F_MUNMAP)) return false;
	if (is_concordant(flag, r.isize, a.mean, a.sd, a.times)) return false;
	const int n = r.nc;
	if (n > 0 && ((cand_op(r, 0) & 15u) == C_H || (cand_op(r, n - 1) & 15u) == C_H)) return false;
	return true;
}

template <typename F, typename H> __device__ __forceinline__ void discordant_walk(const GetsvArgs &a, const CandRec &r, int tid, int pos, int64_t lo, F junction_at, H hit)
{
	const int n = r.nc;
	int rend = pos;
	if (n == 0) rend = pos + 1;
	else for (int k = 0; k < n; ++k) { const uint32_t c = cand_op(r, k); const int op = (int)(c & 15u); if (op == C_M || op == C_D || op == C_N) rend += (int)(c >> 4); }
	for (int64_t m = lo; m < a.n_junc; ++m) {
		const DevJunction j = junction_at(m);
		if (j.up_tid != tid || j.beg >= rend) break;
		if (!(rend > j.beg && pos < j.end)) continue;
		if (discordant_geometry(j, r.flag, pos, r.mpos, r.lq, r.mtid, a.min_ins, a.max_ins)) hit(m, j);
	}
}

__device__ __forceinline__ void discordant_record(const GetsvArgs &a, const CandRec &r, int tid, int pos, int64_t tile)
{
	if (!discordant_read(a, r)) return;
	discordant_walk(a, r, tid, pos, a.tile_junc[tile], [&](int64_t m) { return a.junc[m]; }, [&](int64_t, const DevJunction &j) { atomicAdd(&a.counts[j.orig], 1); });
}

__device__ __forceinline__ void depth_segment(const GetsvArgs &a, int tid, int s, int e, int64_t tile, int64_t &w, int sign)
{
	if (w < 0) w = a.tile_win[tile];
	while (w < a.n_win && a.win_tid[w] == tid && a.win_end[w] < s) ++w;
	for (int64_t x = w; x < a.n_win && a.win_tid[x] == tid && a.win_beg[x] <= e; ++x) {
		int wb = a.win_beg[x], we = a.win_end[x];
		int lo = s > wb ? s : wb, hi = e < we ? e : we;
		int32_t *d = a.diff + a.win_off[x];
		atomicAdd(&d[lo - wb], sign);
		atomicAdd(&d[hi + 1 - wb], -sign);
	}
}

__device__ __forceinline__ bool depth_counts(const GetsvArgs &a, const CandRec &r)
{
	if (r.mapq < a.depth_min_mapq) return false;
	return !(r.flag & (F_UNMAP | F_SECONDARY | F_QCFAIL | F_DUP));
}

__device__ __forceinline__ void depth_record(const GetsvArgs &a, const CandRec &r, int tid, int pos, int64_t tile, int sign = 1)
{
	if (sign > 0 && !depth_counts(a, r)) return;
	const int n = r.nc;
	int col = pos + 1;
	int64_t w = -1;
	for (int k = 0; k < n; ++k) {
		const uint32_t c = cand_op(r, k);
		int op = (int)(c & 15u), len = (int)(c >> 4);
		if (op == C_M) {
			if (len > 0) depth_segment(a, tid, col, col + len - 1, tile, w, sign);
			col += len;
		} else if (op == C_D || op == C_N) col += len;
	}
}

__device__ __forceinline__ uint32_t getsv_tile_bits(const GetsvArgs &a, int tid, int pos, int64_t &tile)
{
	tile = 0;
	if (tid < 0 || tid >= a.n_targets || pos < 0) return 0;
	int64_t t = a.ctg_tile_off[tid] + (pos >> TILE_SHIFT);
	tile = t;
	return t < a.ctg_tile_off[tid + 1] ? a.tilemap[t] : 0u;
}

__global__ void k_tile_mark_windows(const int32_t *__restrict__ win_tid, const int32_t *__restrict__ win_beg, const int32_t *__restrict__ win_end, int64_t n_win, int32_t span,
                                    const int64_t *__restrict__ ctg_tile_off, int32_t n_targets, uint32_t *__restrict__ map32, uint32_t *__restrict__ tile_win)
{
	const int64_t w = (int64_t)blockIdx.x * blockDim.x + threadIdx.x;
	if (w >= n_win) return;
	const int tid = win_tid[w];
	if (tid < 0 || tid >= n_targets) return;
	int64_t p0 = (int64_t)win_beg[w] - span, p1 = (int64_t)win_end[w] - 1;
	if (p1 < 0) return;
	if (p0 < 0) p0 = 0;
	const int64_t base = ctg_tile_off[tid], ntile = ctg_tile_off[tid + 1] - base;
	int64_t t0 = p0 >> TILE_SHIFT, t1 = p1 >> TILE_SHIFT;
	if (t0 >= ntile) return;
	if (t1 >= ntile) t1 = ntile - 1;
	for (int64_t t = t0; t <= t1; ++t) {
		const int col = (int)(t << TILE_SHIFT) + 1;
		int64_t lo = 0, hi = n_win;
		while (lo < hi) {
			const int64_t m = (lo + hi) >> 1;
			const int wt = win_tid[m];
			if (wt < tid || (wt == tid && win_end[m] < col)) lo = m + 1; else hi = m;
		}
		tile_win[base + t] = (uint32_t)lo;
		atomicOr(&map32[(base + t) >> 2], (uint32_t)TM_DEPTH << (8 * ((base + t) & 3)));
	}
}

__global__ void k_tile_mark_junctions(const DevJunction *__restrict__ junc, int64_t n_junc, int32_t span, int32_t wmax, const int64_t *__restrict__ ctg_tile_off, int32_t n_targets,
                                      uint32_t *__restrict__ map32, uint32_t *__restrict__ tile_junc)
{
	const int64_t k = (int64_t)blockIdx.x * blockDim.x + threadIdx.x;
	if (k >= n_junc) return;
	const int tid = junc[k].up_tid;
	if (tid < 0 || tid >= n_targets) return;
	int64_t p0 = (int64_t)junc[k].beg - span, p1 = (int64_t)junc[k].end - 1;
	if (p1 < 0) return;
	if (p0 < 0) p0 = 0;
	const int64_t base = ctg_tile_off[tid], ntile = ctg_tile_off[tid + 1] - base;
	int64_t t0 = p0 >> TILE_SHIFT, t1 = p1 >> TILE_SHIFT;
	if (t0 >= ntile) return;
	if (t1 >= ntile) t1 = ntile - 1;
	for (int64_t t = t0; t <= t1; ++t) {
		const int64_t want = (t << TILE_SHIFT) - (int64_t)wmax;
		int64_t lo = 0, hi = n_junc;
		while (lo < hi) {
			const int64_t m = (lo + hi) >> 1;
			if (junc[m].up_tid < tid || (junc[m].up_tid == tid && (int64_t)junc[m].beg <= want)) lo = m + 1; else hi = m;
		}
		tile_junc[base + t] = (uint32_t)lo;
		atomicOr(&map32[(base + t) >> 2], (uint32_t)TM_JUNC << (8 * ((base + t) & 3)));
	}
}

struct GetsvStage {
	uint32_t *tile_cnt, *tile_off, *stage;
	int64_t block_cap;
	int *overflow;
	int64_t ntiles;
	struct DenseTile *dense_list;
	int *dense_n;
	unsigned long long *n_cand;
};

__device__ __forceinline__ int tile_run_tid(const RunTab &R, int64_t tile, int64_t n)
{
	if (R.n <= 0 || (tile + 1) * CS_TILE > n) return -1;
	const int64_t i0 = tile * CS_TILE, i1 = (tile + 1) * CS_TILE;
	int lo = 0, hi = R.n - 1;
	while (lo < hi) { const int m = (lo + hi + 1) >> 1; if (R.first[m] <= i0) lo = m; else hi = m - 1; }
	return R.first[lo + 1] >= i1 && R.tid[lo] >= 0 ? R.tid[lo] : -1;
}

__device__ __forceinline__ void getsv_scan_load(const DevBatch &b, int64_t tile, int4 (&t4)[CS_SUB], int4 (&p4)[CS_SUB], int run_tid)
{
	const int64_t t0 = tile * CS_TILE + (int64_t)threadIdx.x * CS_ITEMS;
	if (run_tid >= 0) {
#pragma unroll
		for (int sub = 0; sub < CS_SUB; ++sub) {
			t4[sub] = make_int4(run_tid, run_tid, run_tid, run_tid);
			p4[sub] = stream_load_i4(b.pos + t0 + (int64_t)sub * (BLOCK * CS_ITEMS));
		}
	} else if ((tile + 1) * CS_TILE <= b.n) {
#pragma unroll
		for (int sub = 0; sub < CS_SUB; ++sub) {
			t4[sub] = stream_load_i4(b.tid + t0 + (int64_t)sub * (BLOCK * CS_ITEMS));
			p4[sub] = stream_load_i4(b.pos + t0 + (int64_t)sub * (BLOCK * CS_ITEMS));
		}
	} else {
#pragma unroll
		for (int sub = 0; sub < CS_SUB; ++sub) {
			const int64_t i0 = t0 + (int64_t)sub * (BLOCK * CS_ITEMS);
			int tt[CS_ITEMS], pp[CS_ITEMS];
#pragma unroll
			for (int k = 0; k < CS_ITEMS; ++k) { bool in = i0 + k < b.n; tt[k] = in ? b.tid[i0 + k] : -1; pp[k] = in ? b.pos[i0 + k] : 0; }
			t4[sub] = make_int4(tt[0], tt[1], tt[2], tt[3]); p4[sub] = make_int4(pp[0], pp[1], pp[2], pp[3]);
		}
	}
}

__global__ __launch_bounds__(BLOCK) void k_verify_runs(const int32_t *__restrict__ tid, int64_t n, RunTab runs, unsigned long long *bad)
{
	for (int64_t i0 = ((int64_t)blockIdx.x * BLOCK + threadIdx.x) * 4; i0 < n; i0 += (int64_t)gridDim.x * BLOCK * 4) {
		int k = 0;
		while (k + 1 < runs.n && runs.first[k + 1] <= i0) ++k;
		if (i0 + 4 <= n) {
			const int4 t = stream_load_i4(tid + i0);
			const int v[4] = {t.x, t.y, t.z, t.w};
#pragma unroll
			for (int j = 0; j < 4; ++j) {
				while (k + 1 < runs.n && runs.first[k + 1] <= i0 + j) ++k;
				if (v[j] != runs.tid[k]) atomicMax(bad, (unsigned long long)(i0 + j + 1));
			}
		} else for (int64_t i = i0; i < n; ++i) {
			while (k + 1 < runs.n && runs.first[k + 1] <= i) ++k;
			if (tid[i] != runs.tid[k]) atomicMax(bad, (unsigned long long)(i + 1));
		}
	}
}

__global__ __launch_bounds__(BLOCK) void k_getsv_scan(GetsvArgs a, GetsvStage g)
{
	__shared__ uint64_t lds[2][WAVES_PER_BLOCK];
	const DevBatch &b = a.b;
	uint32_t cursor = 0;
	int parity = 0;
	const int64_t region = (int64_t)blockIdx.x * g.block_cap;
	const int last_tid = a.n_targets - 1;
	int4 t4[CS_SUB], p4[CS_SUB], nt4[CS_SUB], np4[CS_SUB];
	int run = -1, nrun = -1;
	if ((int64_t)blockIdx.x < g.ntiles) { run = tile_run_tid(a.runs, blockIdx.x, b.n); getsv_scan_load(b, blockIdx.x, t4, p4, run); }
	for (int64_t tile = blockIdx.x; tile < g.ntiles; tile += gridDim.x, parity ^= 1) {
		const int64_t t0 = tile * CS_TILE + (int64_t)threadIdx.x * CS_ITEMS;
		const int64_t next = tile + gridDim.x;
		if (next < g.ntiles) { nrun = tile_run_tid(a.runs, next, b.n); getsv_scan_load(b, next, nt4, np4, nrun); }
		uint32_t mask = 0;
		const int tid0 = run >= 0 ? run : __builtin_amdgcn_readfirstlane(t4[0].x);
		bool same = true;
		int pmin = 0x7fffffff, pmax = -1;
		if (run >= 0) {
#pragma unroll
			for (int sub = 0; sub < CS_SUB; ++sub) {
				pmin = min(pmin, min(min(p4[sub].x, p4[sub].y), min(p4[sub].z, p4[sub].w)));
				pmax = max(pmax, max(max(p4[sub].x, p4[sub].y), max(p4[sub].z, p4[sub].w)));
			}
			same = pmin >= 0;
		} else {
#pragma unroll
			for (int sub = 0; sub < CS_SUB; ++sub) {
				const int tid[CS_ITEMS] = {t4[sub].x, t4[sub].y, t4[sub].z, t4[sub].w};
				const int pos[CS_ITEMS] = {p4[sub].x, p4[sub].y, p4[sub].z, p4[sub].w};
#pragma unroll
				for (int k = 0; k < CS_ITEMS; ++k) {
					same = same && tid[k] == tid0 && pos[k] >= 0;
					pmin = pos[k] < pmin ? pos[k] : pmin;
					pmax = pos[k] > pmax ? pos[k] : pmax;
				}
			}
		}
		const bool uniform = __all(same) && tid0 >= 0 && tid0 <= last_tid;
		int wmin = 0, wmax = 0;
		if (uniform) {
			const int wpmin = -wave_max(-pmin), wpmax = wave_max(pmax);
			wmin = wpmin >> TILE_SHIFT; wmax = wpmax >> TILE_SHIFT;
			if (a.cap_flag && wpmax - wpmin <= a.cap_span && lane_id() == 0) *a.cap_flag = 1;
		}
		if (uniform && wmax - wmin < WAVE) {
			const int64_t lo = scalar_load(a.ctg_tile_off + tid0), hi = scalar_load(a.ctg_tile_off + tid0 + 1);
			const int64_t mine = lo + wmin + lane_id();
			const uint64_t interesting = __ballot(mine < hi && a.tilemap[mine < hi ? mine : hi - 1] != 0);
			if (interesting) {
#pragma unroll
				for (int sub = 0; sub < CS_SUB; ++sub) {
					const int pos[CS_ITEMS] = {p4[sub].x, p4[sub].y, p4[sub].z, p4[sub].w};
#pragma unroll
					for (int k = 0; k < CS_ITEMS; ++k)
						mask |= ((uint32_t)(interesting >> ((pos[k] >> TILE_SHIFT) - wmin)) & 1u) << (sub * CS_ITEMS + k);
				}
			}
		} else {
#pragma unroll
			for (int sub = 0; sub < CS_SUB; ++sub) {
				const int tid[CS_ITEMS] = {t4[sub].x, t4[sub].y, t4[sub].z, t4[sub].w};
				const int pos[CS_ITEMS] = {p4[sub].x, p4[sub].y, p4[sub].z, p4[sub].w};
#pragma unroll
				for (int k = 0; k < CS_ITEMS; ++k) {
					const int tc = tid[k] < 0 ? 0 : (tid[k] > last_tid ? last_tid : tid[k]);
					const int64_t lo = a.ctg_tile_off[tc], hi = a.ctg_tile_off[tc + 1];
					int64_t t = lo + ((pos[k] < 0 ? 0 : pos[k]) >> TILE_SHIFT);
					const bool valid = tid[k] >= 0 && tid[k] <= last_tid && pos[k] >= 0 && t < hi;
					t = t < hi ? t : hi - 1;
					const bool cand = valid && a.tilemap[t] != 0;
					mask |= (cand ? 1u : 0u) << (sub * CS_ITEMS + k);
				}
			}
		}
		uint64_t packed = 0;
#pragma unroll
		for (int sub = 0; sub < CS_SUB; ++sub) packed |= (uint64_t)__popc((mask >> (sub * CS_ITEMS)) & ((1u << CS_ITEMS) - 1u)) << (16 * sub);
		stage_tile_candidates<CS_ITEMS, true>(mask, packed, tile, t0, lds, parity, cursor, region, g.block_cap, g.tile_cnt, g.tile_off, g.stage, g.overflow);
#pragma unroll
		for (int sub = 0; sub < CS_SUB; ++sub) { t4[sub] = nt4[sub]; p4[sub] = np4[sub]; }
		run = nrun;
	}
	if (g.n_cand && threadIdx.x == 0 && cursor) atomicAdd(g.n_cand, (unsigned long long)cursor);
}

__device__ __forceinline__ void getsv_scan_load_pos(const DevBatch &b, int64_t tile, int4 (&p4)[CS_SUB])
{
	const int64_t t0 = tile * CS_TILE + (int64_t)threadIdx.x * CS_ITEMS;
#pragma unroll
	for (int sub = 0; sub < CS_SUB; ++sub) p4[sub] = stream_load_i4(b.pos + t0 + (int64_t)sub * (BLOCK * CS_ITEMS));
}

constexpr int CS_AHEAD = 2;

__global__ __launch_bounds__(BLOCK, 4) void k_getsv_scan_runs(GetsvArgs a, GetsvStage g)
{
	__shared__ uint64_t lds[2][WAVES_PER_BLOCK];
	__shared__ int s_pos[CS_SUB * CS_ITEMS][BLOCK];
	const DevBatch &b = a.b;
	uint32_t cursor = 0;
	int parity = 0;
	const int64_t region = (int64_t)blockIdx.x * g.block_cap;
	const int last_tid = a.n_targets - 1;
	auto by_record = [&](const int4 (&q)[CS_SUB], int run_, int64_t tile, int64_t t0) -> uint32_t {
		const bool partial = (tile + 1) * CS_TILE > b.n;
#pragma unroll
		for (int sub = 0; sub < CS_SUB; ++sub) {
			s_pos[sub * CS_ITEMS + 0][threadIdx.x] = q[sub].x; s_pos[sub * CS_ITEMS + 1][threadIdx.x] = q[sub].y;
			s_pos[sub * CS_ITEMS + 2][threadIdx.x] = q[sub].z; s_pos[sub * CS_ITEMS + 3][threadIdx.x] = q[sub].w;
		}
		int r = 0;
		if (run_ < 0) { int hi = a.runs.n - 1; const int64_t i0 = tile * CS_TILE; while (r < hi) { const int m = (r + hi + 1) >> 1; if (a.runs.first[m] <= i0) r = m; else hi = m - 1; } }
		uint32_t mask = 0;
#pragma nounroll
		for (int j = 0; j < CS_SUB * CS_ITEMS; ++j) {
			const int64_t i = t0 + (int64_t)(j / CS_ITEMS) * (BLOCK * CS_ITEMS) + (j % CS_ITEMS);
			const int pos = partial ? (i < b.n ? b.pos[i] : 0) : s_pos[j][threadIdx.x];
			int tid = run_;
			if (run_ < 0) {
				while (r + 1 < a.runs.n && a.runs.first[r + 1] <= i) ++r;
				tid = i < b.n ? a.runs.tid[r] : -1;
			}
			const int tc = tid < 0 ? 0 : (tid > last_tid ? last_tid : tid);
			const int64_t lo = a.ctg_tile_off[tc], hi = a.ctg_tile_off[tc + 1];
			int64_t t = lo + ((pos < 0 ? 0 : pos) >> TILE_SHIFT);
			const bool valid = tid >= 0 && tid <= last_tid && pos >= 0 && t < hi;
			t = t < hi ? t : hi - 1;
			if (valid && a.tilemap[t] != 0) mask |= 1u << j;
		}
		return mask;
	};
	constexpr int NB = CS_AHEAD + 1;
	int4 pq[NB][CS_SUB];
	int run = -1, wmin = 0, nrun = -1, nwmin = 0;
	bool fast = false, nfast = false;
	bool cap_seen = false;
	uint8_t tmq[NB];
	bool tm_in = false, ntm_in = false;
	const int full_tiles = __builtin_amdgcn_readfirstlane((int)(b.n / CS_TILE));
	auto head = [&](int64_t tile, const int4 (&q)[CS_SUB], int &run_, bool &fast_, int &wmin_, uint8_t &tm_, bool &in_) {
		run_ = tile < g.ntiles ? tile_run_tid(a.runs, tile, b.n) : -1;
		int pmin = 0x7fffffff, pmax = -1;
#pragma unroll
		for (int sub = 0; sub < CS_SUB; ++sub) {
			pmin = min(pmin, min(min(q[sub].x, q[sub].y), min(q[sub].z, q[sub].w)));
			pmax = max(pmax, max(max(q[sub].x, q[sub].y), max(q[sub].z, q[sub].w)));
		}
		const bool ok = run_ >= 0 && run_ <= last_tid && __all(pmin >= 0);
		const int wpmin = -wave_max(-pmin), wpmax = wave_max(pmax);
		wmin_ = wpmin >> TILE_SHIFT;
		cap_seen = cap_seen || (ok && wpmax - wpmin <= a.cap_span);
		fast_ = ok && (wpmax >> TILE_SHIFT) - wmin_ < WAVE;
		const int rc = ok ? run_ : 0;
		const int64_t lo = scalar_load(a.ctg_tile_off + rc), hi = scalar_load(a.ctg_tile_off + rc + 1);
		const int64_t mine = lo + (fast_ ? wmin_ : 0) + lane_id();
		in_ = fast_ && mine < hi;
		tm_ = a.tilemap[mine < hi ? mine : (hi > 0 ? hi - 1 : 0)];
	};
	auto step = [&](int64_t tile, const int4 (&cur)[CS_SUB], const int4 (&nxt)[CS_SUB], int4 (&far)[CS_SUB], const uint8_t &tm, uint8_t &ntm) {
		const int64_t t0 = tile * CS_TILE + (int64_t)threadIdx.x * CS_ITEMS;
		const int64_t next = tile + gridDim.x;
		const int ahead = (int)tile + CS_AHEAD * (int)gridDim.x;
		getsv_scan_load_pos(b, ahead < full_tiles ? ahead : full_tiles - 1, far);
		head(next, nxt, nrun, nfast, nwmin, ntm, ntm_in);
		uint32_t mask = 0;
		if (fast) {
			const uint64_t interesting = __ballot(tm_in && tm != 0);
			if (interesting) {
#pragma unroll
				for (int sub = 0; sub < CS_SUB; ++sub) {
					const int pos[CS_ITEMS] = {cur[sub].x, cur[sub].y, cur[sub].z, cur[sub].w};
#pragma unroll
					for (int k = 0; k < CS_ITEMS; ++k)
						mask |= ((uint32_t)(interesting >> ((pos[k] >> TILE_SHIFT) - wmin)) & 1u) << (sub * CS_ITEMS + k);
				}
			}
		} else mask = by_record(cur, run, tile, t0);
		uint64_t packed = 0;
#pragma unroll
		for (int sub = 0; sub < CS_SUB; ++sub) packed |= (uint64_t)__popc((mask >> (sub * CS_ITEMS)) & ((1u << CS_ITEMS) - 1u)) << (16 * sub);
		stage_tile_candidates<CS_ITEMS, true>(mask, packed, tile, t0, lds, parity, cursor, region, g.block_cap, g.tile_cnt, g.tile_off, g.stage, g.overflow);
		run = nrun; fast = nfast; wmin = nwmin; tm_in = ntm_in;
		parity ^= 1;
	};
#pragma unroll
	for (int d = 0; d < CS_AHEAD; ++d) { const int t = (int)blockIdx.x + d * (int)gridDim.x; getsv_scan_load_pos(b, t < full_tiles ? t : full_tiles - 1, pq[d]); }
	head(blockIdx.x, pq[0], run, fast, wmin, tmq[0], tm_in);
	int64_t tile = blockIdx.x;
	while (tile < g.ntiles) {
#pragma unroll
		for (int j = 0; j < NB; ++j) {
			if (tile >= g.ntiles) break;
			step(tile, pq[j], pq[(j + 1) % NB], pq[(j + CS_AHEAD) % NB], tmq[j], tmq[(j + 1) % NB]);
			tile += gridDim.x;
		}
	}
	if (g.n_cand && threadIdx.x == 0 && cursor) atomicAdd(g.n_cand, (unsigned long long)cursor);
	if (cap_seen && a.cap_flag && lane_id() == 0) *a.cap_flag = 1;
}

constexpr uint32_t GC_DENSE_MIN = 128;
constexpr int GC_COLS = 4096;

constexpr int GC_NTB = GC_COLS / (1 << TILE_SHIFT) + 1;

struct DenseTile {
	uint32_t so, n;
	int32_t T0, P0;
	int64_t tb0;
	uint32_t jlo, wlo;
	uint8_t tb[GC_NTB + 7 - (GC_NTB + 7) % 8];
};

__global__ __launch_bounds__(BLOCK) void k_dense_tiles(GetsvArgs a, GetsvStage g)
{
	__shared__ int s_w[WAVES_PER_BLOCK + 1];
	const int64_t t = (int64_t)blockIdx.x * BLOCK + threadIdx.x;
	const uint32_t n = t < g.ntiles ? g.tile_cnt[t] : 0u;
	const bool dense = n >= GC_DENSE_MIN;
	int total;
	const int at = block_exclusive_sum<int>(dense ? 1 : 0, s_w, &total);
	if (!total) return;
	if (threadIdx.x == 0) s_w[WAVES_PER_BLOCK] = atomicAdd(g.dense_n, total);
	__syncthreads();
	if (!dense) return;
	DenseTile e;
	e.so = g.tile_off[t]; e.n = n;
	const RecLine l0 = rec_load(a.b.rec, g.stage[e.so]);
	e.T0 = l0.tid(); e.P0 = l0.pos();
	e.tb0 = a.ctg_tile_off[e.T0] + (e.P0 >> TILE_SHIFT);
	const int64_t tb_end = a.ctg_tile_off[e.T0 + 1];
	int dj = -1, dd = -1;
#pragma unroll
	for (int i = GC_NTB - 1; i >= 0; --i) {
		const uint8_t m = e.tb0 + i < tb_end ? a.tilemap[e.tb0 + i] : (uint8_t)0;
		e.tb[i] = m;
		if (m & TM_JUNC) dj = i;
		if (m & TM_DEPTH) dd = i;
	}
	e.jlo = dj >= 0 ? a.tile_junc[e.tb0 + dj] : (uint32_t)a.n_junc;
	e.wlo = dd >= 0 ? a.tile_win[e.tb0 + dd] : (uint32_t)a.n_win;
	g.dense_list[s_w[WAVES_PER_BLOCK] + at] = e;
}

__global__ __launch_bounds__(BLOCK) void k_getsv_cand(GetsvArgs a, GetsvStage g)
{
	const int64_t t0 = (int64_t)blockIdx.x * WAVES_PER_BLOCK;
	uint32_t n[WAVES_PER_BLOCK], so[WAVES_PER_BLOCK], total = 0;
#pragma unroll
	for (int w = 0; w < WAVES_PER_BLOCK; ++w) {
		const bool in = t0 + w < g.ntiles;
		n[w] = in ? g.tile_cnt[t0 + w] : 0u; so[w] = in ? g.tile_off[t0 + w] : 0u;
		if (g.dense_list && n[w] >= GC_DENSE_MIN) n[w] = 0;
		total += n[w];
	}
	const uint32_t c1 = n[0], c2 = c1 + n[1], c3 = c2 + n[2];
	for (uint32_t k = threadIdx.x; k < total; k += BLOCK) {
		const uint32_t at = k < c1 ? so[0] + k : (k < c2 ? so[1] + (k - c1) : (k < c3 ? so[2] + (k - c2) : so[3] + (k - c3)));
		const CandRec r = cand_load(a.b, g.stage[at]);
		const int tid = r.line.tid(), pos = r.line.pos();
		int64_t tile;
		const uint32_t m = getsv_tile_bits(a, tid, pos, tile);
		if (m & TM_JUNC) discordant_record(a, r, tid, pos, tile);
		if (m & TM_DEPTH) depth_record(a, r, tid, pos, tile);
	}
}

constexpr int GC_JC = 32, GC_WC = 16;
constexpr int GC_U = 2;
__global__ __launch_bounds__(BLOCK) void k_getsv_cand_dense(GetsvArgs a, GetsvStage g)
{
	__shared__ int32_t s_l[GC_COLS];
	__shared__ DevJunction s_j[GC_JC];
	__shared__ int32_t s_jc[GC_JC];
	__shared__ int32_t s_wtid[GC_WC], s_wbeg[GC_WC], s_wend[GC_WC];
	__shared__ int64_t s_woff[GC_WC];
	__shared__ uint8_t s_tb[GC_NTB];
	__shared__ int32_t s_chunk[BLOCK];
	__shared__ int32_t s_w[WAVES_PER_BLOCK + 1];
	if ((int)blockIdx.x >= *g.dense_n) return;
	const DenseTile *ep = g.dense_list + blockIdx.x;
	const uint32_t n1 = ep->n, so1 = ep->so;
	CandRec r[GC_U];
#pragma unroll
	for (int u = 0; u < GC_U; ++u) { const uint32_t k = u * BLOCK + threadIdx.x; r[u] = cand_load(a.b, g.stage[so1 + (k < n1 ? k : n1 - 1)]); }
	for (int i = (int)threadIdx.x; i < GC_COLS; i += BLOCK) s_l[i] = 0;
	const int T0 = ep->T0, P0 = ep->P0, C0 = P0 + 1;
	const int64_t tb0 = ep->tb0, jlo = ep->jlo, wlo = ep->wlo;
	if (threadIdx.x < GC_NTB) s_tb[threadIdx.x] = ep->tb[threadIdx.x];
	if (threadIdx.x < GC_JC) { s_jc[threadIdx.x] = 0; if (jlo + threadIdx.x < a.n_junc) s_j[threadIdx.x] = a.junc[jlo + threadIdx.x]; }
	else if (threadIdx.x < GC_JC + GC_WC) {
		const int i = (int)threadIdx.x - GC_JC;
		const int64_t x = wlo + i;
		const bool in = x < a.n_win;
		s_wtid[i] = in ? a.win_tid[x] : -1; s_wbeg[i] = in ? a.win_beg[x] : 0; s_wend[i] = in ? a.win_end[x] : 0; s_woff[i] = in ? a.win_off[x] : 0;
	}
	__syncthreads();
	auto one = [&](const CandRec &r) {
		const int tid = r.line.tid(), pos = r.line.pos();
		int64_t tile;
		uint32_t m;
		const int dt = (pos >> TILE_SHIFT) - (P0 >> TILE_SHIFT);
		const bool here = tid == T0 && pos >= P0 && dt < GC_NTB;
		if (here) { m = s_tb[dt]; tile = tb0 + dt; }
		else m = getsv_tile_bits(a, tid, pos, tile);
		if ((m & TM_JUNC) && discordant_read(a, r)) {
			if (here) discordant_walk(a, r, tid, pos, jlo, [&](int64_t x) { return x - jlo < GC_JC ? s_j[x - jlo] : a.junc[x]; },
			                          [&](int64_t x, const DevJunction &j) { if (x - jlo < GC_JC) atomicAdd(&s_jc[x - jlo], 1); else atomicAdd(&a.counts[j.orig], 1); });
			else discordant_record(a, r, tid, pos, tile);
		}
		if (!(m & TM_DEPTH) || !depth_counts(a, r)) return;
		int col = pos + 1;
		int64_t wcur = -1;
		for (int q = 0; q < r.nc; ++q) {
			const uint32_t c = cand_op(r, q);
			const int op = (int)(c & 15u), len = (int)(c >> 4);
			if (op == C_M) {
				if (len > 0) {
					const int s = col, e = col + len - 1;
					if (tid == T0 && s >= C0 && e + 1 - C0 < GC_COLS) { atomicAdd(&s_l[s - C0], 1); atomicAdd(&s_l[e + 1 - C0], -1); }
					else depth_segment(a, tid, s, e, tile, wcur, 1);
				}
				col += len;
			} else if (op == C_D || op == C_N) col += len;
		}
	};
#pragma unroll
	for (int u = 0; u < GC_U; ++u) if (u * BLOCK + threadIdx.x < n1) one(r[u]);
	for (uint32_t k0 = BLOCK * GC_U; k0 < n1; k0 += BLOCK * GC_U) {
#pragma unroll
		for (int u = 0; u < GC_U; ++u) { const uint32_t k = k0 + u * BLOCK + threadIdx.x; r[u] = cand_load(a.b, g.stage[so1 + (k < n1 ? k : n1 - 1)]); }
#pragma unroll
		for (int u = 0; u < GC_U; ++u) if (k0 + u * BLOCK + threadIdx.x < n1) one(r[u]);
	}
	__syncthreads();
	if (threadIdx.x < GC_JC && s_jc[threadIdx.x]) atomicAdd(&a.counts[s_j[threadIdx.x].orig], s_jc[threadIdx.x]);
	constexpr int PER = GC_COLS / BLOCK;
	int32_t mine = 0;
#pragma unroll 8
	for (int j = 0; j < PER; ++j) mine += s_l[(int)threadIdx.x * PER + j];
	int32_t tot;
	s_chunk[threadIdx.x] = block_exclusive_sum(mine, s_w, &tot);
	__syncthreads();
	auto pre = [&](int c) -> int32_t {
		int32_t v = s_chunk[c / PER];
		for (int j = (c / PER) * PER; j <= c; ++j) v += s_l[j];
		return v;
// ... 276 lines not shown
```

### seeksv_amd/host/bam_reader.cpp

```cpp
#include <sys/mman.h>
#include <sys/stat.h>
#include <unistd.h>

#include "../csrc/cpus.h"
#include "seeksv_host.h"

#include <pthread.h>
#include <zlib.h>

#include "huff_gz.h"

#include <algorithm>
#include <atomic>
#include <cerrno>
#include <chrono>
#include <condition_variable>
#include <cstdio>
#include <cstdlib>
#include <cstring>
#include <functional>
#include <mutex>
#include <new>
#include <string>
#include <thread>
// ... 757 lines not shown
		}
		b->chain_cur = cur;
		return true;
	};
	if (!hop_tail()) return -1;
	while ((int64_t)found.size() < max_records && b->chain_cur < BYTE_LIMIT) {
		if (segs.size() < (size_t)(Bgzf::CHUNK_BLOCKS / Bgzf::SEG_BLOCKS + 1)) segs.resize((size_t)(Bgzf::CHUNK_BLOCKS / Bgzf::SEG_BLOCKS + 1));
		Bgzf *zp = &z;
		const double tg0 = now();
		const int32_t *tlen = b->lens.data();
		const int nseg = z.grow([&segs, zp, n_targets, tlen](int sg, size_t s0, size_t s1) { find_records(zp->ubuf.data(), s0, s1, n_targets, tlen, segs[(size_t)sg]); });
		if (nseg == 0) {
			if (!g_err.empty()) return -1;
			break;
		}
		const double tg1 = now();
		if (timing) fprintf(stderr, "  grow %.4f s nseg %d ulen %zu cap %zu found %zu\n", tg1 - tg0, nseg, z.ulen, z.ubuf.size(), found.size());
		const uint8_t *u = z.ubuf.data();
		size_t cur = b->chain_cur;
		bool window_end = false;
		for (int sg = 0; sg < nseg && !window_end; ++sg) {
			const Segment &S = segs[(size_t)sg];
			while (cur < S.end) {
				size_t k = 0;
				if (S.list.empty() || S.list[0] != cur) k = (size_t)(std::lower_bound(S.list.begin(), S.list.end(), cur) - S.list.begin());
				if (k < S.list.size() && S.list[k] == cur) { found.insert(found.end(), S.list.begin() + (ptrdiff_t)k, S.list.end()); cur = S.exit; break; }
				uint32_t bs;
				if (cur + 4 > z.ulen) { window_end = true; break; }
				memcpy(&bs, u + cur, 4);
				if (bs < 32) { g_err = "corrupt BAM record"; return -1; }
				if (cur + 4 + (size_t)bs > z.ulen) { window_end = true; break; }
				found.push_back(cur);
				cur += 4 + (size_t)bs;
			}
		}
		while (!found.empty()) {
			uint32_t bs; memcpy(&bs, u + found.back(), 4);
			if (found.back() + 4 + (size_t)bs <= z.ulen) break;
			cur = found.back(); found.pop_back();
		}
		b->chain_cur = cur;
		if (!hop_tail()) return -1;
	}
	if (z.eof && g_err.empty() && (int64_t)found.size() < max_records && b->chain_cur != z.ulen) { g_err = "truncated BAM record"; return -1; }
	const double t1 = now();
	const int64_t n = std::min<int64_t>((int64_t)found.size(), max_records);
	const std::vector<size_t> &off = found;
	const uint8_t *base = z.ubuf.data();
	B.tid.resize((size_t)n); B.pos.resize((size_t)n); B.l_qseq.resize((size_t)n); B.mtid.resize((size_t)n); B.mpos.resize((size_t)n); B.isize.resize((size_t)n);
	B.flag.resize((size_t)n); B.n_cigar.resize((size_t)n); B.mapq.resize((size_t)n); B.xc.resize((size_t)n); B.ends.resize((size_t)n); B.cigar_off.resize((size_t)n); B.seq_off.resize((size_t)n);
	const int nt = (int)std::min<int64_t>(std::max<int64_t>(1, n / 8192), 128);
	std::vector<uint64_t> c_of((size_t)nt + 1, 0), s_of((size_t)nt + 1, 0);
	std::atomic<int> bad{0};
	pool().run(nt, [&](int t) {
		const int64_t i0 = n * t / nt, i1 = n * (t + 1) / nt;
		uint64_t ct = 0, st = 0;
		for (int64_t i = i0; i < i1; ++i) {
			const uint8_t *r = base + off[(size_t)i] + 4;
			uint32_t bs; memcpy(&bs, r - 4, 4);
			uint16_t ncig; int32_t l_seq;
			memcpy(&ncig, r + 12, 2); memcpy(&l_seq, r + 16, 4);
			const size_t o_cig = 32 + (size_t)r[8];
			if (l_seq < 0 || o_cig + 4 * (size_t)ncig + ((size_t)l_seq + 1) / 2 + (size_t)l_seq > (size_t)bs) { bad.store(1); return; }
			bool soft = false;
			if (ncig) {
				uint32_t c0, cl; memcpy(&c0, r + o_cig, 4); memcpy(&cl, r + o_cig + 4 * ((size_t)ncig - 1), 4);
				soft = (c0 & 15) == 4 || (cl & 15) == 4;
			}
			ct += ncig;
			if (soft || keep_all_seq) st += ((size_t)l_seq + 1) / 2 + (size_t)l_seq;
		}
		c_of[(size_t)t + 1] = ct; s_of[(size_t)t + 1] = st;
	});
	if (bad.load()) { g_err = "corrupt BAM record"; return -1; }
	for (int t = 0; t < nt; ++t) { c_of[(size_t)t + 1] += c_of[(size_t)t]; s_of[(size_t)t + 1] += s_of[(size_t)t]; }
	const uint64_t ctot = c_of[(size_t)nt], stot = s_of[(size_t)nt];
	if (ctot > 0xffffffffull) { g_err = "too many CIGAR operations in one batch"; return -1; }
	if (B.cigar.size() < (size_t)ctot + 1) B.cigar.resize((size_t)ctot + 1);
	if (B.seqqual.size() < (size_t)stot + 16) B.seqqual.resize((size_t)stot + 16);
	const double t2 = now();
	std::vector<int64_t> span_of((size_t)nt, 1);
	std::vector<std::vector<uint8_t>> un((size_t)nt);
	pool().run(nt, [&](int t) {
		const int64_t i0 = n * t / nt, i1 = n * (t + 1) / nt;
		int64_t max_span = 1;
		uint64_t c_run = c_of[(size_t)t], s_run = s_of[(size_t)t];
		for (int64_t i = i0; i < i1; ++i) {
			const uint8_t *r = base + off[(size_t)i] + 4;
			uint32_t bs; memcpy(&bs, r - 4, 4);
			int32_t refid, pos, l_seq, next_ref, next_pos, tlen;
			uint16_t ncig, flag;
			memcpy(&refid, r, 4); memcpy(&pos, r + 4, 4);
			const uint8_t l_read_name = r[8], mapq = r[9];
			memcpy(&ncig, r + 12, 2); memcpy(&flag, r + 14, 2); memcpy(&l_seq, r + 16, 4);
			memcpy(&next_ref, r + 20, 4); memcpy(&next_pos, r + 24, 4); memcpy(&tlen, r + 28, 4);
			const size_t o_name = 32, o_cig = o_name + l_read_name, o_seq = o_cig + 4 * (size_t)ncig;
			const size_t o_qual = o_seq + ((size_t)l_seq + 1) / 2, o_aux = o_qual + (size_t)l_seq;
			B.tid[(size_t)i] = refid; B.pos[(size_t)i] = pos; B.flag[(size_t)i] = flag; B.mapq[(size_t)i] = mapq; B.n_cigar[(size_t)i] = ncig;
			B.l_qseq[(size_t)i] = l_seq; B.mtid[(size_t)i] = next_ref; B.mpos[(size_t)i] = next_pos; B.isize[(size_t)i] = tlen;
			uint32_t *cd = B.cigar.data() + c_run;
			B.cigar_off[(size_t)i] = (uint32_t)c_run; c_run += ncig;
			if (ncig) memcpy(cd, r + o_cig, 4 * (size_t)ncig);
			int64_t span = 0;
			for (unsigned k = 0; k < ncig; ++k) { unsigned op = cd[k] & 15; if (op == 0 || op == 2 || op == 3 || op == 7 || op == 8) span += cd[k] >> 4; }
			if (span > max_span) max_span = span;
			const bool soft = ncig && ((cd[0] & 15) == 4 || (cd[ncig - 1] & 15) == 4);
			B.ends[(size_t)i] = ncig ? (uint8_t)((cd[0] & 15u) | ((cd[ncig - 1] & 15u) << 4)) : (uint8_t)0xff;
			B.xc[(size_t)i] = soft ? (uint8_t)(aux_xc(r + o_aux, r + bs) != 0) : (uint8_t)0;
			if (soft || keep_all_seq) {
				B.seq_off[(size_t)i] = s_run;
				memcpy(B.seqqual.data() + s_run, r + o_seq, o_aux - o_seq);
				s_run += o_aux - o_seq;
			} else B.seq_off[(size_t)i] = SSV_NO_SEQ;
			if (flag & (4 | 8)) {
				un[(size_t)t].insert(un[(size_t)t].end(), r - 4, r + bs);
			}
		}
		span_of[(size_t)t] = max_span;
	});
	int64_t max_span = 1;
	{ size_t total = 0; for (auto &u : un) total += u.size(); B.unmapped_raw.reserve(total); }
	for (int t = 0; t < nt; ++t) {
		max_span = std::max(max_span, span_of[(size_t)t]);
		B.unmapped_raw.insert(B.unmapped_raw.end(), un[(size_t)t].begin(), un[(size_t)t].end());
	}
	if (b->keep_names) {
		B.name_off.resize((size_t)n + 1);
		uint64_t tot = 0;
		for (int64_t i = 0; i < n; ++i) { B.name_off[(size_t)i] = tot; tot += base[off[(size_t)i] + 4 + 8]; }
		B.name_off[(size_t)n] = tot;
		B.names.resize((size_t)tot + 1);
		pool().run(nt, [&](int t) {
			for (int64_t i = n * t / nt, i1 = n * (t + 1) / nt; i < i1; ++i) {
				const uint8_t *r = base + off[(size_t)i] + 4;
				const size_t ln = r[8];
				char *dst = B.names.data() + B.name_off[(size_t)i];
				memcpy(dst, r + 32, ln);
				if (ln) dst[ln - 1] = 0;
			}
		});
	}
	if (timing) fprintf(stderr, "[read_batch] n=%lld inflate+find %.3f s, sizes %.3f s, decode %.3f s, window %zu MB\n", (long long)n, t1 - t0, t2 - t1, now() - t2, z.ulen >> 20);
	b->found_pos = (size_t)n;
	z.upos = (size_t)n < found.size() ? found[(size_t)n] : b->chain_cur;
	memset(out, 0, sizeof(*out));
	out->n = n; out->mem = SSV_MEM_HOST;
	out->max_ref_span = (int32_t)(max_span > INT32_MAX ? INT32_MAX : max_span);
	out->tid = B.tid.data(); out->pos = B.pos.data(); out->flag = B.flag.data(); out->mapq = B.mapq.data();
	out->n_cigar = B.n_cigar.data(); out->l_qseq = B.l_qseq.data(); out->mtid = B.mtid.data(); out->mpos = B.mpos.data();
	out->isize = B.isize.data(); out->cigar_off = B.cigar_off.data(); out->cigar = B.cigar.data(); out->xc = B.xc.data();
	out->seq_off = B.seq_off.data(); out->seqqual = B.seqqual.data(); out->cigar_ends = B.ends.data();
	out->n_cigar_total = (int64_t)ctot; out->seqqual_bytes = (int64_t)stot;
	B.tid_runs.clear();
	for (int64_t i = 0; i < n && B.tid_runs.size() <= 64; ++i)
		if (i == 0 || B.tid.data()[i] != B.tid.data()[i - 1]) B.tid_runs.push_back(ssv_tid_run{i, B.tid.data()[i], 0});
	if (!B.tid_runs.empty() && B.tid_runs.size() <= 64) { out->tid_runs = B.tid_runs.data(); out->n_tid_runs = (int64_t)B.tid_runs.size(); }
	return 0;
}

int ssvh_bam_read_batch(ssvh_bam *b, int64_t max_records, int keep_all_seq, ssv_batch_t *out)
{
	if (!b->readahead) { b->cur = 0; return decode_batch(b, b->buf[0], max_records, keep_all_seq, out); }
	int rc;
	if (b->ra_thread.joinable()) {
		b->ra_thread.join();
		if (b->ra_max != max_records || b->ra_keep != keep_all_seq) { g_err = "read-ahead is on: every ssvh_bam_read_batch call must ask for the same batch"; return -1; }
		b->cur = (b->cur + 1) % 3;
		rc = b->ra_rc; g_err = b->ra_err; *out = b->ra_batch;
	} else rc = decode_batch(b, b->buf[b->cur], max_records, keep_all_seq, out);
	if (rc == 0 && out->n > 0) {
		b->ra_max = max_records; b->ra_keep = keep_all_seq;
		b->ra_thread = std::thread([b] {
			b->ra_rc = decode_batch(b, b->buf[(b->cur + 1) % 3], b->ra_max, b->ra_keep, &b->ra_batch);
			b->ra_err = g_err;
		});
	}
	return rc;
}

int ssvh_bam_set_allocator(ssvh_bam *b, void *(*alloc)(size_t), void (*release)(void *))
{
	if (b->ra_thread.joinable()) { g_err = "a read-ahead is in flight"; return -1; }
	b->alloc.alloc = alloc; b->alloc.release = release;
	for (auto &B : b->buf) B.use(&b->alloc);
	return 0;
}

int ssvh_bam_keep_names(ssvh_bam *b, int on)
{
	if (b->ra_thread.joinable()) { g_err = "a read-ahead is in flight"; return -1; }
	b->keep_names = on != 0;
	return 0;
}

int ssvh_bam_batch_names(const ssvh_bam *b, ssv_names_t *out)
{
	if (!out) { g_err = "ssvh_bam_batch_names: no output"; return -1; }
	if (!b->keep_names) { g_err = "ssvh_bam_batch_names: names are not kept (ssvh_bam_keep_names)"; return -1; }
	const ssvh_bam::BatchBuf &B = b->buf[b->cur];
	memset(out, 0, sizeof(*out));
	out->mem = SSV_MEM_HOST;
	out->base = B.names.data(); out->off = B.name_off.data();
	out->bytes = B.name_off.empty() ? 0 : (int64_t)B.name_off.back();
	return 0;
}

int ssvh_bam_set_readahead(ssvh_bam *b, int on)
{
	if (b->ra_thread.joinable()) { g_err = "a read-ahead is in flight"; return -1; }
	b->readahead = on != 0;
	return 0;
}

int ssvh_bam_next_record(ssvh_bam *b, ssvh_record *out)
{
	g_err.clear();
	if (b->ra_thread.joinable()) { g_err = "a read-ahead is in flight: record-at-a-time reads cannot be mixed in"; return -1; }
	b->found.clear(); b->found_pos = 0;
	int32_t block_size;
	const uint8_t *r;
	if (b->z.ulen - b->z.upos >= 4 && (memcpy(&block_size, b->z.ubuf.data() + b->z.upos, 4), block_size >= 32) && b->z.ulen - b->z.upos - 4 >= (size_t)block_size) {
		r = b->z.ubuf.data() + b->z.upos + 4;
		b->z.upos += 4 + (size_t)block_size;
	} else {
		size_t got = b->z.read(&block_size, 4);
		if (got == 0) return g_err.empty() ? 0 : -1;
		if (got != 4 || block_size < 32) { if (g_err.empty()) g_err = "truncated BAM record"; return -1; }
		b->rec.resize((size_t)block_size + 4);
		if (b->z.read(b->rec.data(), (size_t)block_size) != (size_t)block_size) { if (g_err.empty()) g_err = "truncated BAM record"; return -1; }
		r = b->rec.data();
	}
	memcpy(&out->tid, r, 4); memcpy(&out->pos, r + 4, 4);
	const uint8_t l_read_name = r[8];
	out->mapq = r[9];
	memcpy(&out->n_cigar, r + 12, 2); memcpy(&out->flag, r + 14, 2); memcpy(&out->l_qseq, r + 16, 4);
	const size_t o_cig = 32 + (size_t)l_read_name, o_seq = o_cig + 4 * (size_t)out->n_cigar, o_qual = o_seq + ((size_t)out->l_qseq + 1) / 2;
	if (out->l_qseq < 0 || o_qual + (size_t)out->l_qseq > (size_t)block_size) { g_err = "corrupt BAM record"; return -1; }
	out->qname = (const char *)r + 32;
	if (out->n_cigar <= 8) {
		if (out->n_cigar) memcpy(b->small_cigar, r + o_cig, 4 * (size_t)out->n_cigar);
		out->cigar = b->small_cigar;
	} else {
		b->buf[0].cigar.assign((size_t)out->n_cigar, 0);
		memcpy(b->buf[0].cigar.data(), r + o_cig, 4 * (size_t)out->n_cigar);
		out->cigar = b->buf[0].cigar.data();
	}
	out->seq = r + o_seq; out->qual = r + o_qual;
	return 1;
}


static int bgzf_level()
{
	const char *e = getenv("SSV_BGZF_LEVEL");
	const int l = e ? atoi(e) : 1;
	return l < -2 ? -2 : l > 9 ? 9 : l;
}

static void bgzf_compress_blocks(const std::vector<uint8_t> &raw, std::vector<uint8_t> &out)
{
	const size_t BS = 0xff00;
	const size_t nb = (raw.size() + BS - 1) / BS;
	std::vector<std::vector<uint8_t>> comp(nb);
	const int level = bgzf_level();
	wpool().run((int)nb, [&](int i) {
		const size_t off = (size_t)i * BS, len = std::min(BS, raw.size() - off);
		std::vector<uint8_t> &c = comp[(size_t)i];
		const uint8_t hdr[16] = {31, 139, 8, 4, 0, 0, 0, 0, 0, 255, 6, 0, 66, 67, 2, 0};
		if (level < 0) {
			static thread_local std::vector<uint8_t> room;
			if (room.size() < ssvh_huff::member_bound(BS)) room.resize(ssvh_huff::member_bound(BS));
			size_t clen = (size_t)((level == -2 ? ssvh_huff::deflate_fast(raw.data() + off, len, room.data()) : ssvh_huff::deflate_literals(raw.data() + off, len, room.data())) - room.data());
			if (clen > len + 5) {
				uint8_t *p = room.data();
				const uint16_t l16 = (uint16_t)len, n16 = (uint16_t)~l16;
				p[0] = 1; memcpy(p + 1, &l16, 2); memcpy(p + 3, &n16, 2); memcpy(p + 5, raw.data() + off, len);
				clen = len + 5;
			}
			c.resize(18 + clen + 8);
			memcpy(c.data(), hdr, 16);
			const uint16_t bsize = (uint16_t)(clen + 25);
			memcpy(c.data() + 16, &bsize, 2);
			memcpy(c.data() + 18, room.data(), clen);
			const uint32_t crc = (uint32_t)crc32(crc32(0L, Z_NULL, 0), raw.data() + off, (uInt)len), isz = (uint32_t)len;
			memcpy(c.data() + 18 + clen, &crc, 4); memcpy(c.data() + 18 + clen + 4, &isz, 4);
			return;
		}
		c.resize(len + 1024);
		struct Deflater { z_stream zs; int level = -1; ~Deflater() { if (level >= 0) deflateEnd(&zs); } };
		static thread_local Deflater D;
		if (D.level != level) {
			if (D.level >= 0) deflateEnd(&D.zs);
			memset(&D.zs, 0, sizeof(D.zs));
			deflateInit2(&D.zs, level, Z_DEFLATED, -15, 8, Z_DEFAULT_STRATEGY);
			D.level = level;
		} else deflateReset(&D.zs);
		z_stream &zs = D.zs;
		zs.next_in = const_cast<uint8_t *>(raw.data() + off); zs.avail_in = (uInt)len;
		zs.next_out = c.data() + 18; zs.avail_out = (uInt)(c.size() - 18 - 8);
		deflate(&zs, Z_FINISH);
		size_t clen = zs.total_out;
		memcpy(c.data(), hdr, 16);
		uint16_t bsize = (uint16_t)(clen + 25);
		memcpy(c.data() + 16, &bsize, 2);
		uint32_t crc = (uint32_t)crc32(crc32(0L, Z_NULL, 0), raw.data() + off, (uInt)len), isz = (uint32_t)len;
		memcpy(c.data() + 18 + clen, &crc, 4); memcpy(c.data() + 18 + clen + 4, &isz, 4);
		c.resize(18 + clen + 8);
	});
// ... 225 lines not shown
```

### seeksv_amd/synth.py

```python
import ctypes as C
import math
import os

import numpy as np

from . import _abi

HG38 = [248956422, 242193529, 198295559, 190214555, 181538259, 170805979, 159345973, 145138636, 138394717, 133797422, 135086622,
        133275309, 114364328, 107043718, 101991189, 90338345, 83257441, 80373285, 58617616, 64444167, 46709983, 50818468, 156040895, 57227415]
HG38_NAMES = [f"chr{i}" for i in range(1, 23)] + ["chrX", "chrY"]
SEED = 0x5EE45F
MAX_CONTIGS = 64


class SyConfig(C.Structure):
    _fields_ = [("seed", C.c_uint64), ("n_total", C.c_int64), ("n_contigs", C.c_int32), ("read_len", C.c_int32),
                ("contig_off", C.c_int64 * (MAX_CONTIGS + 1)), ("contig_len", C.c_int32 * MAX_CONTIGS), ("spacing_fp", C.c_uint64),
                ("clip_permille", C.c_int32), ("indel_permille", C.c_int32), ("dup_permille", C.c_int32), ("sec_permille", C.c_int32),
                ("improper_permille", C.c_int32), ("vaf_permille", C.c_int32), ("n_breakends", C.c_int32), ("qual_model", C.c_int32), ("unmap_permille", C.c_int32)]


BREAKEND_DTYPE = np.dtype([("lin", np.int64), ("tid", np.int32), ("q", np.int32), ("ptid", np.int32), ("ppos", np.int32),
                           ("side", np.int8), ("pdir", np.int8), ("mate_rev", np.int8), ("is_up", np.int8), ("mate_anchor", np.int32)])
assert BREAKEND_DTYPE.itemsize == 32
# ... 119 lines not shown
                A = int(rng2.randint(1500, self.lens[ta] - 1500))
                if made == 0:
                    B = int(rng2.randint(40, 190))
                elif made == 1:
                    B = int(rng2.randint(hl - 190, hl - 40))
                else:
                    B = int(rng2.randint(200, hl - 200))
                if not free(ta, A) or any(abs(B - u) < 40 for u in used_b):
                    continue
                take(ta, A); used_b.add(B)
                la = int(self.offs[ta])
                kind = made % 4
                if kind == 0:
                    junctions.append((self.names[ta], A, "+", "HBV", B, "+"))
                    be.append((la + A, ta, A, tb, B - 1, 0, 1, 1, 1, B - 1))
                    be.append((lb + B - 1, tb, B - 1, ta, A - 1, 1, -1, 0, 0, 0))
                elif kind == 1:
                    junctions.append(("HBV", B, "+", self.names[ta], A, "+"))
                    be.append((lb + B, tb, B, ta, A - 1, 0, 1, 1, 1, A - 1))
                    be.append((la + A - 1, ta, A - 1, tb, B - 1, 1, -1, 0, 0, 0))
                elif kind == 2:
                    junctions.append((self.names[ta], A, "+", "HBV", B, "-"))
                    be.append((la + A, ta, A, tb, B - 1, 0, -1, 0, 1, B - 1))
                    be.append((lb + B, tb, B, ta, A - 1, 0, -1, 0, 0, 0))
                else:
                    junctions.append((self.names[ta], A, "-", "HBV", B, "+"))
                    be.append((la + A - 1, ta, A - 1, tb, B - 1, 1, 1, 1, 1, B - 1))
                    be.append((lb + B - 1, tb, B - 1, ta, A - 1, 1, 1, 0, 0, 0))
                made += 1
        arr = np.array(be, dtype=BREAKEND_DTYPE) if be else np.zeros(0, dtype=BREAKEND_DTYPE)
        self.breakends = np.sort(arr, order="lin")
        self.junctions = sorted(junctions, key=lambda j: (j[0], j[3], j[2], j[5], j[1], j[4]))

    def reference_fasta(self):
        lib = _lib(False)
        lib.ssvs_ref_bases.argtypes = [C.POINTER(SyConfig), C.c_int32, C.c_int64, C.c_int64, C.c_char_p]
        out = []
        for tid, (name, ln) in enumerate(zip(self.names, self.lens)):
            buf = C.create_string_buffer(int(ln))
            lib.ssvs_ref_bases(C.byref(self.cfg), tid, 0, int(ln), buf)
            seq = buf.raw.decode()
            out.append(f">{name}\n" + "\n".join(seq[i:i + 80] for i in range(0, len(seq), 80)) + "\n")
        return "".join(out)

    def write_fasta(self, path, threads=8):
        from concurrent.futures import ThreadPoolExecutor
        lib = _lib(False)
        lib.ssvs_ref_bases.argtypes = [C.POINTER(SyConfig), C.c_int32, C.c_int64, C.c_int64, C.c_void_p]
        PIECE = 8_000_000

        def piece(args):
            tid, start, n = args
            buf = np.empty(n, np.uint8)
            lib.ssvs_ref_bases(C.byref(self.cfg), tid, start, n, buf.ctypes.data)
            full = n // 80 * 80
            body = np.empty((full // 80, 81), np.uint8)
            body[:, :80] = buf[:full].reshape(-1, 80)
            body[:, 80] = 10
            return body.tobytes() + buf[full:].tobytes() + (b"\n" if n > full else b"")
        with open(path, "wb") as f, ThreadPoolExecutor(max_workers=max(1, threads)) as ex:
            for tid, (name, ln) in enumerate(zip(self.names, self.lens)):
                f.write(f">{name}\n".encode())
                for chunk in ex.map(piece, [(tid, s, min(PIECE, int(ln) - s)) for s in range(0, int(ln), PIECE)]):
                    f.write(chunk)

    def reference_2bit(self, device=None):
        n_words = (self.genome_len + 31) // 32 + 1
        off = np.asarray(self.offs, np.int64)
        if device is None:
            lib = _lib(False)
            out = np.zeros(n_words, np.uint64)
            lib.ssvs_ref_2bit(C.byref(self.cfg), C.c_void_p(out.ctypes.data), C.c_int64(n_words))
            return out, off
        import torch
        lib = _lib(True)
        torch.cuda.set_device(device)
        out = torch.zeros(n_words, dtype=torch.int64, device=torch.device("cuda", device))
        if lib.ssvs_ref_2bit(C.byref(self.cfg), C.c_void_p(out.data_ptr()), C.c_int64(n_words)) != 0:
            raise RuntimeError("ssvs_ref_2bit: " + lib.ssvs_last_error().decode())
        return out, off

    def generate_host(self, g0, n, with_rec=False, all_seq=False):
        lib = _lib(False)
        be = self.breakends
        bep = be.ctypes.data if len(be) else None
        a = dict(n_cigar=np.zeros(n, np.uint16), cigar_off=np.zeros(n, np.uint32), seq_off=np.zeros(n, np.uint64))
        nct, sqb = C.c_int64(), C.c_int64()
        p = lambda x: x.ctypes.data if x.size else None
        lib.ssvs_plan(C.byref(self.cfg), bep, g0, n, p(a["n_cigar"]), p(a["cigar_off"]), p(a["seq_off"]), C.byref(nct), C.byref(sqb))
        for name, dt in (("tid", np.int32), ("pos", np.int32), ("flag", np.uint16), ("mapq", np.uint8), ("l_qseq", np.int32),
                         ("mtid", np.int32), ("mpos", np.int32), ("isize", np.int32)):
            a[name] = np.zeros(n, dt)
        a["cigar"] = np.zeros(nct.value, np.uint32)
        a["seqqual"] = np.zeros(sqb.value, np.uint8)
        rec = np.zeros(n, _abi.RECORD_DTYPE) if with_rec else None
        a["cigar_ends"] = np.zeros(n, np.uint8)
        lib.ssvs_fill(C.byref(self.cfg), bep, g0, n, p(a["tid"]), p(a["pos"]), p(a["flag"]), p(a["mapq"]), p(a["n_cigar"]), p(a["l_qseq"]),
                      p(a["mtid"]), p(a["mpos"]), p(a["isize"]), p(a["cigar_off"]), p(a["cigar"]), p(a["seq_off"]), p(a["seqqual"]),
                      p(rec) if with_rec else None, p(a["cigar_ends"]))
        if with_rec:
            a["rec"] = rec
        if all_seq:
            entry = (self.read_len + 1) // 2 + self.read_len
            a["seqqual"] = np.empty(n * entry + 16, np.uint8)
            a["seq_off"] = (np.arange(n, dtype=np.uint64) * np.uint64(entry))
            lib.ssvs_fill_seq_all(C.byref(self.cfg), bep, C.c_int64(g0), C.c_int64(n), p(a["seqqual"]))
            a["seqqual_bytes"] = n * entry
        a["xc"] = None
        a["max_ref_span"] = self.max_ref_span
        return a

    def generate_device(self, g0, n, device, soa=True, persistent=False):
        import torch
        lib = _lib(True)
        torch.cuda.set_device(device)
        dev = torch.device("cuda", device)
        if device not in self._be_dev:
            be = self.breakends
            self._be_dev[device] = torch.from_numpy(be.view(np.uint8).copy()).to(dev) if len(be) else torch.zeros(32, dtype=torch.uint8, device=dev)
        bep = self._be_dev[device].data_ptr()
        t = dict(n_cigar=torch.empty(n, dtype=torch.int16, device=dev), cigar_off=torch.empty(n, dtype=torch.int32, device=dev),
                 seq_off=torch.empty(n, dtype=torch.int64, device=dev))
        nct, sqb = C.c_int64(), C.c_int64()
        torch.cuda.synchronize(dev)
        rc = lib.ssvs_plan(C.byref(self.cfg), bep, g0, n, t["n_cigar"].data_ptr(), t["cigar_off"].data_ptr(), t["seq_off"].data_ptr(), C.byref(nct), C.byref(sqb))
        if rc != 0:
            raise RuntimeError("ssvs_plan: " + lib.ssvs_last_error().decode())
        cold = (("flag", torch.int16), ("mapq", torch.uint8), ("l_qseq", torch.int32), ("mtid", torch.int32), ("mpos", torch.int32), ("isize", torch.int32))
        for name, dt in (("tid", torch.int32), ("pos", torch.int32)) + (cold if soa else ()):
            t[name] = torch.empty(n, dtype=dt, device=dev)
        t["cigar"] = torch.empty(max(nct.value, 4), dtype=torch.int32, device=dev)
        t["seqqual"] = torch.empty(sqb.value + 16, dtype=torch.uint8, device=dev)
        t["rec"] = torch.empty(max(n, 1) * 64, dtype=torch.uint8, device=dev)
        t["cigar_ends"] = torch.empty(n + 16, dtype=torch.uint8, device=dev)
        ptr = lambda k: t[k].data_ptr() if k in t else None
        rc = lib.ssvs_fill(C.byref(self.cfg), bep, g0, n, ptr("tid"), ptr("pos"), ptr("flag"), ptr("mapq"),
                           ptr("n_cigar"), ptr("l_qseq"), ptr("mtid"), ptr("mpos"), ptr("isize"),
                           ptr("cigar_off"), ptr("cigar"), ptr("seq_off"), ptr("seqqual"), ptr("rec"), ptr("cigar_ends"))
        if rc != 0:
            raise RuntimeError("ssvs_fill: " + lib.ssvs_last_error().decode())
        if not soa:
            del t["cigar_off"], t["seq_off"]
        arrays = {k: v.data_ptr() for k, v in t.items()}
        arrays["xc"] = None
        arrays["n_cigar_total"] = nct.value
        arrays["seqqual_bytes"] = sqb.value
        arrays["max_ref_span"] = self.max_ref_span
        if n > 1:
            tt = t["tid"]
            ch = (torch.nonzero(tt[1:] != tt[:-1]).flatten() + 1).cpu().numpy()
            starts = np.concatenate(([0], ch)).astype(np.int64)
            runs = np.zeros(len(starts), _abi.TID_RUN_DTYPE)
            runs["first"], runs["tid"] = starts, tt[torch.from_numpy(starts).to(dev)].cpu().numpy()
            arrays["tid_runs"] = runs
        elif n == 1:
            runs = np.zeros(1, _abi.TID_RUN_DTYPE)
            runs["tid"] = int(t["tid"][0].item())
            arrays["tid_runs"] = runs
        b, _ = _abi.make_batch(arrays, mem=_abi.MEM_DEVICE | (_abi.MEM_PERSISTENT if persistent else 0), n=n)
        return b, t
```

Measured before the change: 62.46 billion.

## Skip getsv scan tiles whose sorted position range covers no marked tiles

Adds a per-run position-sorted flag to tid_runs, filled by the BAM decoder, host reader and synthetic generator. When a run is flagged sorted, a prefix sum over the tilemap lets a new pre-pass mark each scan tile live only if its position span overlaps a marked reference tile. A compaction kernel then builds a list of live tiles, and the scan kernel walks only that list. This avoids scanning records that cannot produce candidates, at the cost of two extra kernel launches, a tilemap prefix scan, and an ABI field change from pad to flags.

```diff
diff --git a/include/seeksv_hip.h b/include/seeksv_hip.h
--- a/include/seeksv_hip.h
+++ b/include/seeksv_hip.h
@@ -66,7 +66,8 @@
 	int64_t n_tid_runs;
 } ssv_batch_t;
 
-typedef struct ssv_tid_run { int64_t first; int32_t tid; int32_t pad; } ssv_tid_run;
+typedef struct ssv_tid_run { int64_t first; int32_t tid; int32_t flags;  } ssv_tid_run;
+#define SSV_RUN_POS_SORTED 1
 
 typedef struct ssv_ctx ssv_ctx;
 
diff --git a/seeksv_amd/_abi.py b/seeksv_amd/_abi.py
--- a/seeksv_amd/_abi.py
+++ b/seeksv_amd/_abi.py
@@ -39,7 +39,8 @@
         return np.frombuffer((C.c_uint8 * (16 * self.n_tid_runs)).from_address(self.tid_runs), dtype=TID_RUN_DTYPE).copy()
 
 
-TID_RUN_DTYPE = np.dtype([("first", np.int64), ("tid", np.int32), ("pad", np.int32)])
+TID_RUN_DTYPE = np.dtype([("first", np.int64), ("tid", np.int32), ("flags", np.int32)])
+RUN_POS_SORTED = 1
 
 
 def runs_of_tid(tid):
diff --git a/seeksv_amd/csrc/bamdec_api.inc b/seeksv_amd/csrc/bamdec_api.inc
--- a/seeksv_amd/csrc/bamdec_api.inc
+++ b/seeksv_amd/csrc/bamdec_api.inc
@@ -338,7 +338,7 @@
 	const uint32_t run_cap = 1u << 16;
 	CHECK(ensure_up(d.runs, (size_t)run_cap * sizeof(ssv::TidRun)));
 	constexpr uint32_t RAW_RUN_CAP = 64;
-	CHECK(ensure_up(d.raw_runs, (size_t)RAW_RUN_CAP * sizeof(ssv::TidRun))); CHECK(ensure_host(c, d.h_raw_runs, (size_t)RAW_RUN_CAP * sizeof(ssv::TidRun)));
+	CHECK(ensure_up(d.raw_runs, (size_t)2 * RAW_RUN_CAP * sizeof(ssv::TidRun))); CHECK(ensure_host(c, d.h_raw_runs, (size_t)2 * RAW_RUN_CAP * sizeof(ssv::TidRun)));
 	HIPCHECK(c, hipMemsetAsync(d.small.p, 0, 256, st));
 	uint32_t *sm = P<uint32_t>(d.small);
 	{
@@ -368,8 +368,8 @@
 		hipLaunchKernelGGL(ssv::k_tid_tile_last, dim3((unsigned)n_tiles), dim3(BLOCK), 0, st, col.tid, col.flag, n, P<int32_t>(d.tile_last));
 		hipLaunchKernelGGL(ssv::k_tid_tile_carry, dim3(1), dim3(WAVE), 0, st, P<int32_t>(d.tile_last), n_tiles, d.prev_tid, P<int32_t>(d.tile_prev), reinterpret_cast<int32_t *>(sm + 3));
 		hipLaunchKernelGGL(ssv::k_tid_runs, dim3((unsigned)n_tiles), dim3(BLOCK), 0, st, col.tid, col.flag, n, P<int32_t>(d.tile_prev), P<ssv::TidRun>(d.runs), run_cap, sm + 2);
-		hipLaunchKernelGGL(ssv::k_tid_raw_runs, dim3((unsigned)n_tiles), dim3(BLOCK), 0, st, col.tid, n, P<ssv::TidRun>(d.raw_runs), RAW_RUN_CAP, sm + 11);
-		HIPCHECK(c, hipMemcpyAsync(d.h_raw_runs.p, d.raw_runs.p, (size_t)RAW_RUN_CAP * sizeof(ssv::TidRun), hipMemcpyDeviceToHost, st));
+		hipLaunchKernelGGL(ssv::k_tid_raw_runs, dim3((unsigned)n_tiles), dim3(BLOCK), 0, st, col.tid, col.pos, n, P<ssv::TidRun>(d.raw_runs), RAW_RUN_CAP, sm + 11, sm + 12);
+		HIPCHECK(c, hipMemcpyAsync(d.h_raw_runs.p, d.raw_runs.p, (size_t)2 * RAW_RUN_CAP * sizeof(ssv::TidRun), hipMemcpyDeviceToHost, st));
 	}
 	HIPCHECK(c, hipMemcpyAsync(d.h_small.p, d.small.p, 64, hipMemcpyDeviceToHost, st));
 	HIPCHECK(c, hipStreamSynchronize(st));
@@ -404,6 +404,15 @@
 			const ssv::TidRun *r = P<ssv::TidRun>(d.h_raw_runs);
 			for (uint32_t k = 0; k < nr; ++k) d.tid_runs.push_back(ssv_tid_run{(int64_t)r[k].index, r[k].tid, 0});
 			std::sort(d.tid_runs.begin(), d.tid_runs.end(), [](const ssv_tid_run &a, const ssv_tid_run &b) { return a.first < b.first; });
+			const uint32_t n_down = hs[12];
+			if (n_down <= RAW_RUN_CAP) {
+				for (ssv_tid_run &x : d.tid_runs) x.flags = SSV_RUN_POS_SORTED;
+				for (uint32_t k = 0; k < n_down; ++k) {
+					const int64_t i = (int64_t)r[RAW_RUN_CAP + k].index;
+					auto it = std::upper_bound(d.tid_runs.begin(), d.tid_runs.end(), i, [](int64_t v, const ssv_tid_run &x) { return v < x.first; });
+					(it - 1)->flags = 0;
+				}
+			}
 			out->tid_runs = d.tid_runs.data(); out->n_tid_runs = (int64_t)nr;
 		}
 	}
diff --git a/seeksv_amd/csrc/bamdec_kernels.h b/seeksv_amd/csrc/bamdec_kernels.h
--- a/seeksv_amd/csrc/bamdec_kernels.h
+++ b/seeksv_amd/csrc/bamdec_kernels.h
@@ -592,7 +592,8 @@
 struct TidRun { uint32_t index; int32_t tid; };
 constexpr int32_t TID_NONE = INT32_MIN;
 
-__global__ __launch_bounds__(BLOCK) void k_tid_raw_runs(const int32_t *__restrict__ tid, int64_t n, TidRun *__restrict__ runs, uint32_t cap, uint32_t *__restrict__ count)
+__global__ __launch_bounds__(BLOCK) void k_tid_raw_runs(const int32_t *__restrict__ tid, const int32_t *__restrict__ pos, int64_t n, TidRun *__restrict__ runs, uint32_t cap,
+                                                       uint32_t *__restrict__ count, uint32_t *__restrict__ n_down)
 {
 	const int64_t i = (int64_t)blockIdx.x * BLOCK + threadIdx.x;
 	if (i >= n) return;
@@ -600,6 +601,9 @@
 	if (i == 0 || tid[i - 1] != t) {
 		const uint32_t k = atomicAdd(count, 1u);
 		if (k < cap) { runs[k].index = (uint32_t)i; runs[k].tid = t; }
+	} else if (pos[i] < pos[i - 1]) {
+		const uint32_t k = atomicAdd(n_down, 1u);
+		if (k < cap) { runs[cap + k].index = (uint32_t)i; runs[cap + k].tid = t; }
 	}
 }
 
diff --git a/seeksv_amd/csrc/getsv_api.inc b/seeksv_amd/csrc/getsv_api.inc
--- a/seeksv_amd/csrc/getsv_api.inc
+++ b/seeksv_amd/csrc/getsv_api.inc
@@ -7,10 +7,12 @@
 	std::vector<int32_t> tlen;
 	std::vector<int64_t> ctg_tile_off;
 	int32_t map_span = -1;
+	int32_t pfx_span = -2;
 	int32_t wmax = 0;
 	int64_t diff_len = 0;
 	DBuf djunc, counts, wtid, wbeg, wend, woff, diff, tilemap, tile_win, tile_junc, ctgoff, maxdepth, span;
 	DBuf q_tid, q_out64;
+	DBuf tile_pfx, pfx_sums, live_flag, live_cnt, live;
 	DBuf dense_list, cap_flags, cap_deep, cap_carry, cap_ring, cap_ring_tmp, cap_tail[2][4];
 	int32_t cap_tail_n = 0, cap_tail_cur = 0, cap_ring_mask = 0;
 	HBuf h_q;
@@ -26,6 +28,7 @@
 		if (i && b->tid_runs[i].first <= b->tid_runs[i - 1].first) { c->err = "tid_runs must be strictly increasing"; return SSV_E_ARG; }
 		if (b->tid_runs[i].first >= b->n) { c->err = "tid_runs reach past the batch"; return SSV_E_ARG; }
 		R.first[i] = b->tid_runs[i].first; R.tid[i] = b->tid_runs[i].tid;
+		if (b->tid_runs[i].flags & SSV_RUN_POS_SORTED) R.sorted |= 1ull << i;
 	}
 	R.first[k] = b->n; R.n = (int32_t)k;
 	return SSV_OK;
@@ -47,6 +50,17 @@
 	return SSV_OK;
 }
 
+static int gs_build_tile_pfx(ssv_ctx *c)
+{
+	ssv_getsv_state &G = *c->getsv;
+	const int64_t ntile = G.ctg_tile_off.back();
+	CHECK(ensure(c, G.tile_pfx, (size_t)(ntile + 1) * 4 + 16)); CHECK(ensure(c, G.pfx_sums, (size_t)scan_scratch_elems(ntile + 1) * 4 + 16));
+	exclusive_scan<TileMarked, uint32_t>(c->st, P<TileMarked>(G.tilemap), P<uint32_t>(G.tile_pfx), ntile + 1, 0u, P<uint32_t>(G.pfx_sums), nullptr);
+	HIPCHECK(c, hipGetLastError());
+	G.pfx_span = G.map_span;
+	return SSV_OK;
+}
+
 int ssv_getsv_begin(ssv_ctx *c, const ssv_getsv_params *p)
 {
 	if (!c || !p || p->n_targets < 0 || p->n_junctions < 0 || p->n_windows < 0) return SSV_E_ARG;
@@ -58,7 +72,7 @@
 	G.tlen.assign(p->target_len, p->target_len + p->n_targets);
 	G.ctg_tile_off.assign((size_t)p->n_targets + 1, 0);
 	for (int t = 0; t < p->n_targets; ++t) G.ctg_tile_off[(size_t)t + 1] = G.ctg_tile_off[(size_t)t] + ((int64_t)std::max(0, G.tlen[(size_t)t]) >> TILE_SHIFT) + 1;
-	G.map_span = -1;
+	G.map_span = -1; G.pfx_span = -2;
 	G.junc.clear();
 	G.wmax = 0;
 	for (int64_t k = 0; k < p->n_junctions; ++k) {
@@ -169,11 +183,14 @@
 		CHECK(ensure_host(c, c->h_counters, sizeof(ClipCounters)));
 		HIPCHECK(c, hipMemsetAsync(c->counters.p, 0, sizeof(ClipCounters), c->st));
 		k_verify_runs<<<(unsigned)std::min<int64_t>(256 * 8, (d.n + BLOCK * 4 - 1) / (BLOCK * 4)), BLOCK, 0, c->st>>>(d.tid, d.n, a.runs, &P<ClipCounters>(c->counters)->n_cand);
+		if (a.runs.sorted) k_verify_sorted<<<(unsigned)std::min<int64_t>(256 * 8, (d.n + BLOCK - 1) / BLOCK), BLOCK, 0, c->st>>>(d.pos, d.n, a.runs, &P<ClipCounters>(c->counters)->n_new);
 		HIPCHECK(c, hipGetLastError());
 		HIPCHECK(c, hipMemcpyAsync(c->h_counters.p, c->counters.p, sizeof(ClipCounters), hipMemcpyDeviceToHost, c->st));
 		HIPCHECK(c, hipStreamSynchronize(c->st));
 		const unsigned long long badrec = P<ClipCounters>(c->h_counters)->n_cand;
 		if (badrec) { c->err = "tid_runs disagree with the tid column at record " + std::to_string(badrec - 1) + " (SSV_VERIFY_RUNS)"; return SSV_E_ARG; }
+		const unsigned long long badpos = P<ClipCounters>(c->h_counters)->n_new;
+		if (badpos) { c->err = "a run of tid_runs is flagged SSV_RUN_POS_SORTED, but record " + std::to_string(badpos - 1) + " starts before its predecessor (SSV_VERIFY_RUNS)"; return SSV_E_ARG; }
 	}
 	a.b = d; a.tilemap = P<uint8_t>(G.tilemap); a.tile_win = P<uint32_t>(G.tile_win); a.tile_junc = P<uint32_t>(G.tile_junc); a.ctg_tile_off = P<int64_t>(G.ctgoff); a.n_targets = G.p.n_targets;
 	a.junc = P<DevJunction>(G.djunc); a.n_junc = (int64_t)G.junc.size(); a.junc_wmax = G.wmax;
@@ -194,7 +211,11 @@
 	if (c->stage_cap == 0) c->stage_cap = std::max<int64_t>(1 << 16, d.n / 8);
 	ClipCounters *hc = P<ClipCounters>(c->h_counters);
 	ClipCounters *dc = P<ClipCounters>(c->counters);
+	const bool walk_live = a.runs.n > 0 && a.runs.sorted != 0 && d.n >= CS_TILE && !getenv("SSV_NO_LIVE_TILES");
+	const unsigned live_blocks = grid_for(ntiles, BLOCK);
+	if (walk_live) { CHECK(ensure(c, G.live_flag, (size_t)ntiles + 16)); CHECK(ensure(c, G.live_cnt, (size_t)live_blocks * 4 + 16)); CHECK(ensure(c, G.live, (size_t)(ntiles + 4 * (int64_t)grid) * 4 + 16)); }
 	GetsvStage g;
+	g.live = nullptr; g.n_live = nullptr;
 	for (int attempt = 0;; ++attempt) {
 		const int64_t block_cap = (c->stage_cap + grid - 1) / grid;
 		CHECK(ensure(c, c->stage, (size_t)block_cap * grid * 4));
@@ -204,7 +225,14 @@
 		g.dense_list = nullptr; g.dense_n = nullptr; g.n_cand = &dc->n_cand;
 		{
 			ProfScope ps(c, P_GETSV_SCAN, d.n);
-			if (a.runs.n > 0 && d.n >= CS_TILE) k_getsv_scan_runs<<<grid, BLOCK, 0, c->st>>>(a, g);
+			if (walk_live && attempt == 0) {
+				if (G.pfx_span != G.map_span) CHECK(gs_build_tile_pfx(c));
+				g.live = P<uint32_t>(G.live); g.n_live = P<int>(G.cap_flags) + 3;
+				k_live_tiles<<<live_blocks, BLOCK, 0, c->st>>>(a, g, P<uint32_t>(G.tile_pfx), P<uint8_t>(G.live_flag), P<uint32_t>(G.live_cnt));
+				k_live_list<<<live_blocks, BLOCK, 0, c->st>>>(P<uint8_t>(G.live_flag), P<uint32_t>(G.live_cnt), ntiles, P<uint32_t>(G.live), P<int>(G.cap_flags) + 3);
+			}
+			if (walk_live) k_getsv_scan_runs<true><<<grid, BLOCK, 0, c->st>>>(a, g);
+			else if (a.runs.n > 0 && d.n >= CS_TILE) k_getsv_scan_runs<false><<<grid, BLOCK, 0, c->st>>>(a, g);
 			else k_getsv_scan<<<grid, BLOCK, 0, c->st>>>(a, g);
 		}
 		HIPCHECK(c, hipGetLastError());
@@ -213,6 +241,11 @@
 		if (!hc->overflow) break;
 		if (attempt > 6) { c->err = "getsv staging overflow"; return SSV_E_HIP; }
 		c->stage_cap *= 4;
+	}
+	if (walk_live && getenv("SSV_LIVE_TILES_REPORT")) {
+		int n_live = 0;
+		HIPCHECK(c, hipMemcpy(&n_live, P<int>(G.cap_flags) + 3, 4, hipMemcpyDeviceToHost));
+		fprintf(stderr, "ssv_getsv_scan: %d of %lld scan tiles live\n", n_live, (long long)ntiles);
 	}
 	{
 		ProfScope ps(c, P_GETSV_CAND, d.n);
diff --git a/seeksv_amd/csrc/getsv_kernels.h b/seeksv_amd/csrc/getsv_kernels.h
--- a/seeksv_amd/csrc/getsv_kernels.h
+++ b/seeksv_amd/csrc/getsv_kernels.h
@@ -91,6 +91,7 @@
 	int32_t n;
 	int32_t tid[RUN_MAX];
 	int64_t first[RUN_MAX + 1];
+	uint64_t sorted;
 };
 
 struct GetsvArgs {
@@ -304,6 +305,8 @@
 	int64_t block_cap;
 	int *overflow;
 	int64_t ntiles;
+	const uint32_t *live;
+	const int *n_live;
 	struct DenseTile *dense_list;
 	int *dense_n;
 	unsigned long long *n_cand;
@@ -363,6 +366,72 @@
 			if (tid[i] != runs.tid[k]) atomicMax(bad, (unsigned long long)(i + 1));
 		}
 	}
+}
+
+__global__ __launch_bounds__(BLOCK) void k_verify_sorted(const int32_t *__restrict__ pos, int64_t n, RunTab runs, unsigned long long *bad)
+{
+	for (int64_t i = (int64_t)blockIdx.x * BLOCK + threadIdx.x + 1; i < n; i += (int64_t)gridDim.x * BLOCK) {
+		bool flagged = false;
+		for (int k = 0; k < runs.n; ++k) flagged = flagged || (runs.first[k] < i && i < runs.first[k + 1] && ((runs.sorted >> k) & 1ull));
+		if (flagged && pos[i] < pos[i - 1]) atomicMax(bad, (unsigned long long)(i + 1));
+	}
+}
+
+struct TileMarked {
+	uint8_t v;
+	__device__ __forceinline__ operator uint32_t() const { return v != 0 ? 1u : 0u; }
+};
+
+constexpr int CAP_SHARE_LO = (WAVES_PER_BLOCK - 1) * WAVE * CS_ITEMS, CAP_SHARE_HI = CS_TILE - 1 - CAP_SHARE_LO;
+
+__global__ __launch_bounds__(BLOCK) void k_live_tiles(GetsvArgs a, GetsvStage g, const uint32_t *__restrict__ tile_pfx, uint8_t *__restrict__ live_flag, uint32_t *__restrict__ block_cnt)
+{
+	__shared__ int s_w[WAVES_PER_BLOCK + 1];
+	const int64_t t = (int64_t)blockIdx.x * BLOCK + threadIdx.x;
+	const int64_t i0 = t * CS_TILE, i1 = i0 + CS_TILE;
+	bool live = t < g.ntiles;
+	if (live && i1 <= a.b.n) {
+		int tid = -1;
+		for (int k = 0; k < a.runs.n; ++k) if (a.runs.first[k] <= i0 && i1 <= a.runs.first[k + 1] && ((a.runs.sorted >> k) & 1ull)) tid = a.runs.tid[k];
+		if (tid >= 0 && tid < a.n_targets) {
+			const int p0 = a.b.pos[i0], p1 = a.b.pos[i1 - 1];
+			const int q0 = a.cap_flag ? a.b.pos[i0 + CAP_SHARE_LO] : 0, q1 = a.cap_flag ? a.b.pos[i0 + CAP_SHARE_HI] : 0;
+			if (p0 >= 0 && p1 >= p0) {
+				const int64_t base = a.ctg_tile_off[tid], nt = a.ctg_tile_off[tid + 1] - base;
+				const int64_t t0 = p0 >> TILE_SHIFT;
+				int64_t t1 = p1 >> TILE_SHIFT;
+				if (t1 >= nt) t1 = nt - 1;
+				live = t0 <= t1 && tile_pfx[base + t1 + 1] != tile_pfx[base + t0];
+				if (!live) {
+					g.tile_cnt[t] = 0;
+					if (a.cap_flag && q1 - q0 <= a.cap_span) *a.cap_flag = 1;
+				}
+			}
+		}
+	}
+	if (t < g.ntiles) live_flag[t] = live ? 1 : 0;
+	int total;
+	block_exclusive_sum<int>(live ? 1 : 0, s_w, &total);
+	if (threadIdx.x == 0) block_cnt[blockIdx.x] = (uint32_t)total;
+}
+
+__global__ __launch_bounds__(BLOCK) void k_live_list(const uint8_t *__restrict__ live_flag, const uint32_t *__restrict__ block_cnt, int64_t ntiles, uint32_t *__restrict__ live, int *__restrict__ n_live)
+{
+	__shared__ int s_w[WAVES_PER_BLOCK + 1];
+	__shared__ int s_before[WAVES_PER_BLOCK];
+	int before = 0;
+	for (int i = threadIdx.x; i < (int)blockIdx.x; i += BLOCK) before += (int)block_cnt[i];
+	before = wave_sum(before);
+	if (lane_id() == 0) s_before[wave_id()] = before;
+	const int64_t t = (int64_t)blockIdx.x * BLOCK + threadIdx.x;
+	const bool is_live = t < ntiles && live_flag[t] != 0;
+	int total;
+	const int at = block_exclusive_sum<int>(is_live ? 1 : 0, s_w, &total);
+	int pre = 0;
+#pragma unroll
+	for (int w = 0; w < WAVES_PER_BLOCK; ++w) pre += s_before[w];
+	if (is_live) live[pre + at] = (uint32_t)t;
+	if (blockIdx.x == gridDim.x - 1 && threadIdx.x == 0) *n_live = pre + total;
 }
 
 __global__ __launch_bounds__(BLOCK) void k_getsv_scan(GetsvArgs a, GetsvStage g)
@@ -461,7 +530,7 @@
 
 constexpr int CS_AHEAD = 2;
 
-__global__ __launch_bounds__(BLOCK, 4) void k_getsv_scan_runs(GetsvArgs a, GetsvStage g)
+template <bool LIVE> __global__ __launch_bounds__(BLOCK, 4) void k_getsv_scan_runs(GetsvArgs a, GetsvStage g)
 {
 	__shared__ uint64_t lds[2][WAVES_PER_BLOCK];
 	__shared__ int s_pos[CS_SUB * CS_ITEMS][BLOCK];
@@ -525,10 +594,8 @@
 		in_ = fast_ && mine < hi;
 		tm_ = a.tilemap[mine < hi ? mine : (hi > 0 ? hi - 1 : 0)];
 	};
-	auto step = [&](int64_t tile, const int4 (&cur)[CS_SUB], const int4 (&nxt)[CS_SUB], int4 (&far)[CS_SUB], const uint8_t &tm, uint8_t &ntm) {
+	auto step = [&](int64_t tile, int64_t next, int ahead, const int4 (&cur)[CS_SUB], const int4 (&nxt)[CS_SUB], int4 (&far)[CS_SUB], const uint8_t &tm, uint8_t &ntm) {
 		const int64_t t0 = tile * CS_TILE + (int64_t)threadIdx.x * CS_ITEMS;
-		const int64_t next = tile + gridDim.x;
-		const int ahead = (int)tile + CS_AHEAD * (int)gridDim.x;
 		getsv_scan_load_pos(b, ahead < full_tiles ? ahead : full_tiles - 1, far);
 		head(next, nxt, nrun, nfast, nwmin, ntm, ntm_in);
 		uint32_t mask = 0;
@@ -551,16 +618,39 @@
 		run = nrun; fast = nfast; wmin = nwmin; tm_in = ntm_in;
 		parity ^= 1;
 	};
-#pragma unroll
-	for (int d = 0; d < CS_AHEAD; ++d) { const int t = (int)blockIdx.x + d * (int)gridDim.x; getsv_scan_load_pos(b, t < full_tiles ? t : full_tiles - 1, pq[d]); }
-	head(blockIdx.x, pq[0], run, fast, wmin, tmq[0], tm_in);
-	int64_t tile = blockIdx.x;
-	while (tile < g.ntiles) {
-#pragma unroll
-		for (int j = 0; j < NB; ++j) {
-			if (tile >= g.ntiles) break;
-			step(tile, pq[j], pq[(j + 1) % NB], pq[(j + CS_AHEAD) % NB], tmq[j], tmq[(j + 1) % NB]);
-			tile += gridDim.x;
+	if constexpr (LIVE) {
+		static_assert(CS_AHEAD == 2, "the walk keeps the tile numbers of this step, the next and the one after in three scalars");
+		const int none = (int)g.ntiles;
+		const int n_live = scalar_load(g.n_live);
+		auto live_at = [&](int k) -> int { return k < n_live ? (int)scalar_load(g.live + k) : none; };
+		const int G = (int)gridDim.x;
+		int k = (int)blockIdx.x;
+		int t_cur = live_at(k), t_nxt = live_at(k + G), t_far = live_at(k + 2 * G);
+		getsv_scan_load_pos(b, t_cur < full_tiles ? t_cur : full_tiles - 1, pq[0]);
+		getsv_scan_load_pos(b, t_nxt < full_tiles ? t_nxt : full_tiles - 1, pq[1]);
+		head(t_cur, pq[0], run, fast, wmin, tmq[0], tm_in);
+		while (t_cur < none) {
+#pragma unroll
+			for (int j = 0; j < NB; ++j) {
+				if (t_cur >= none) break;
+				const int t_new = live_at(k + 3 * G);
+				step(t_cur, t_nxt, t_far, pq[j], pq[(j + 1) % NB], pq[(j + CS_AHEAD) % NB], tmq[j], tmq[(j + 1) % NB]);
+				t_cur = t_nxt; t_nxt = t_far; t_far = t_new;
+				k += G;
+			}
+		}
+	} else {
+#pragma unroll
+		for (int d = 0; d < CS_AHEAD; ++d) { const int t = (int)blockIdx.x + d * (int)gridDim.x; getsv_scan_load_pos(b, t < full_tiles ? t : full_tiles - 1, pq[d]); }
+		head(blockIdx.x, pq[0], run, fast, wmin, tmq[0], tm_in);
+		int64_t tile = blockIdx.x;
+		while (tile < g.ntiles) {
+#pragma unroll
+			for (int j = 0; j < NB; ++j) {
+				if (tile >= g.ntiles) break;
+				step(tile, tile + gridDim.x, (int)tile + CS_AHEAD * (int)gridDim.x , pq[j], pq[(j + 1) % NB], pq[(j + CS_AHEAD) % NB], tmq[j], tmq[(j + 1) % NB]);
+				tile += gridDim.x;
+			}
 		}
 	}
 	if (g.n_cand && threadIdx.x == 0 && cursor) atomicAdd(g.n_cand, (unsigned long long)cursor);
diff --git a/seeksv_amd/host/bam_reader.cpp b/seeksv_amd/host/bam_reader.cpp
--- a/seeksv_amd/host/bam_reader.cpp
+++ b/seeksv_amd/host/bam_reader.cpp
@@ -933,8 +933,10 @@
 	out->seq_off = B.seq_off.data(); out->seqqual = B.seqqual.data(); out->cigar_ends = B.ends.data();
 	out->n_cigar_total = (int64_t)ctot; out->seqqual_bytes = (int64_t)stot;
 	B.tid_runs.clear();
-	for (int64_t i = 0; i < n && B.tid_runs.size() <= 64; ++i)
-		if (i == 0 || B.tid.data()[i] != B.tid.data()[i - 1]) B.tid_runs.push_back(ssv_tid_run{i, B.tid.data()[i], 0});
+	for (int64_t i = 0; i < n && B.tid_runs.size() <= 64; ++i) {
+		if (i == 0 || B.tid.data()[i] != B.tid.data()[i - 1]) B.tid_runs.push_back(ssv_tid_run{i, B.tid.data()[i], SSV_RUN_POS_SORTED});
+		else if (B.pos.data()[i] < B.pos.data()[i - 1]) B.tid_runs.back().flags = 0;
+	}
 	if (!B.tid_runs.empty() && B.tid_runs.size() <= 64) { out->tid_runs = B.tid_runs.data(); out->n_tid_runs = (int64_t)B.tid_runs.size(); }
 	return 0;
 }
diff --git a/seeksv_amd/synth.py b/seeksv_amd/synth.py
--- a/seeksv_amd/synth.py
+++ b/seeksv_amd/synth.py
@@ -295,10 +295,18 @@
             starts = np.concatenate(([0], ch)).astype(np.int64)
             runs = np.zeros(len(starts), _abi.TID_RUN_DTYPE)
             runs["first"], runs["tid"] = starts, tt[torch.from_numpy(starts).to(dev)].cpu().numpy()
+            pp, unsorted = t["pos"], np.zeros(len(starts), bool)
+            for lo in range(0, n - 1, 1 << 26):
+                hi = min(n - 1, lo + (1 << 26))
+                down = torch.nonzero(pp[lo + 1:hi + 1] < pp[lo:hi]).flatten().cpu().numpy() + lo + 1
+                k = np.searchsorted(starts, down, side="right") - 1
+                unsorted[k[starts[k] != down]] = True
+            runs["flags"] = np.where(unsorted, 0, _abi.RUN_POS_SORTED)
             arrays["tid_runs"] = runs
         elif n == 1:
             runs = np.zeros(1, _abi.TID_RUN_DTYPE)
             runs["tid"] = int(t["tid"][0].item())
+            runs["flags"] = _abi.RUN_POS_SORTED
             arrays["tid_runs"] = runs
         b, _ = _abi.make_batch(arrays, mem=_abi.MEM_DEVICE | (_abi.MEM_PERSISTENT if persistent else 0), n=n)
         return b, t
```

Result: no change. 62.64 billion (median of 6 runs) (+0.3%).
